# tpoisonooo/how-to-optimize-gemm

Hardware: NVIDIA B200
Metric: SGEMM GFLOP/s (square N=4096 point of the 256..4096 sweep) (higher is better)
Workload: dtype f16x2(scaled split-f32)

## Files before the change

### how-to-optimize-gemm_b200/csrc/capi.cu

```cuda
#include "../../include/b200gemm.h"

#include <cuda.h>
#include <cuda_runtime.h>
#include <stdio.h>
#include <stdlib.h>
#include <string.h>

#include <atomic>
#include <mutex>
#include <vector>

#include "gemm_ffma.cuh"
#include "gemm_generic.cuh"
#include "gemm_mxf4.cuh"
#include "gemm_tc.cuh"

using namespace b200;

namespace {

std::atomic<unsigned long long> g_launches{0};
int g_split_tail = 1;

struct KernelTimer {
  static constexpr int CAP = 1024;
  bool on = false;
  int n = 0;
  cudaEvent_t ev[CAP][2] = {};
  void begin(cudaStream_t st) {
    if (!on || n >= CAP) return;
    if (!ev[n][0]) { cudaEventCreate(&ev[n][0]); cudaEventCreate(&ev[n][1]); }
    cudaEventRecord(ev[n][0], st);
  }
  void end(cudaStream_t st) {
    if (!on || n >= CAP) return;
    cudaEventRecord(ev[n][1], st);
    n++;
  }
} g_ktimer;
std::atomic<int> g_default_f32_mode{-1};
thread_local const char* t_last_kernel = "none";
struct EpiOpts { int axpby = 0; float alpha = 1.f, beta = 0.f; };
thread_local EpiOpts t_epi;
thread_local int t_sm_reserve = 0;
thread_local int t_dynamic_sched = 0;
int g_dbg_b_lbo = 0, g_dbg_b_sbo = 0;

struct Scratch { void* p = nullptr; size_t bytes = 0; };
struct HostPipe {
  bool ready = false;
  cudaStream_t h2d = nullptr, comp = nullptr, d2h = nullptr;
  cudaEvent_t in[8] = {}, done[8] = {};
  cudaError_t init() {
    if (ready) return cudaSuccess;
    cudaError_t e;
    if ((e = cudaStreamCreateWithFlags(&h2d, cudaStreamNonBlocking)) != cudaSuccess) return e;
    if ((e = cudaStreamCreateWithFlags(&comp, cudaStreamNonBlocking)) != cudaSuccess) return e;
    if ((e = cudaStreamCreateWithFlags(&d2h, cudaStreamNonBlocking)) != cudaSuccess) return e;
    for (int i = 0; i < 8; i++) {
      if ((e = cudaEventCreateWithFlags(&in[i], cudaEventDisableTiming)) != cudaSuccess) return e;
      if ((e = cudaEventCreateWithFlags(&done[i], cudaEventDisableTiming)) != cudaSuccess) return e;
    }
    ready = true;
    return cudaSuccess;
  }
};
struct DevCtx {
  int ok = 0;
  int sms = 0;
  int dev = -1;
  int* flags = nullptr;
  unsigned flag_slot = 0;
  int* sched_counters = nullptr;
  unsigned sched_slot = 0;
  std::mutex ws_mu;
  Scratch ws;
  cudaEvent_t ws_event = nullptr;
  cudaStream_t ws_stream = nullptr;
  bool ws_busy = false;
  unsigned cmax_slot = 0;
  float* cmax_buf = nullptr;
  size_t cmax_cap = 0;
  int cmax_dirty[2] = {0, 0};
  cudaStream_t aux = nullptr;
  cudaEvent_t aux_fork = nullptr, aux_join = nullptr;
  std::mutex host_mu;
  Scratch scr[4];
  HostPipe pipe;
  std::vector<const void*> attr_done;
};
constexpr int kMaxDevices = 64;
DevCtx g_ctx[kMaxDevices];
std::mutex g_mu;

typedef CUresult (*EncodeTiledFn)(CUtensorMap*, CUtensorMapDataType, cuuint32_t, void*,
                                  const cuuint64_t*, const cuuint64_t*, const cuuint32_t*,
                                  const cuuint32_t*, CUtensorMapInterleave, CUtensorMapSwizzle,
                                  CUtensorMapL2promotion, CUtensorMapFloatOOBfill);
EncodeTiledFn g_encode = nullptr;

thread_local DevCtx* t_ctx = nullptr;

int ensure_device() {
  int dev = -1;
  if (cudaGetDevice(&dev) != cudaSuccess || dev < 0 || dev >= kMaxDevices) { cudaGetLastError(); t_ctx = nullptr; return B200_ERR_NO_DEVICE; }
  DevCtx* c = &g_ctx[dev];
  t_ctx = c;
  if (c->ok == 1) return 0;
  std::lock_guard<std::mutex> lk(g_mu);
  if (c->ok == 1) return 0;
  cudaDeviceProp prop;
  if (cudaGetDeviceProperties(&prop, dev) != cudaSuccess) { cudaGetLastError(); c->ok = -1; return B200_ERR_NO_DEVICE; }
  if (prop.major != 10) { c->ok = -1; return B200_ERR_NO_DEVICE; }
  if (!g_encode) {
    void* fn = nullptr;
    cudaDriverEntryPointQueryResult qres;
    if (cudaGetDriverEntryPoint("cuTensorMapEncodeTiled", &fn, cudaEnableDefault, &qres) != cudaSuccess ||
        qres != cudaDriverEntryPointSuccess || !fn) {
      cudaGetLastError();
      c->ok = -1;
      return B200_ERR_NO_DEVICE;
    }
    g_encode = reinterpret_cast<EncodeTiledFn>(fn);
  }
  if (!c->flags) {
    if (cudaMalloc(&c->flags, 16 * 1024 * sizeof(int)) != cudaSuccess || cudaMemset(c->flags, 0, 16 * 1024 * sizeof(int)) != cudaSuccess) {
      cudaGetLastError(); c->flags = nullptr; c->ok = -1; return B200_ERR_NO_DEVICE;
    }
  }
  if (!c->sched_counters) {
    if (cudaMalloc(&c->sched_counters, 64 * sizeof(int)) != cudaSuccess || cudaMemset(c->sched_counters, 0, 64 * sizeof(int)) != cudaSuccess) {
      cudaGetLastError(); c->sched_counters = nullptr; c->ok = -1; return B200_ERR_NO_DEVICE;
    }
  }
  if (!c->ws_event && cudaEventCreateWithFlags(&c->ws_event, cudaEventDisableTiming) != cudaSuccess) {
    cudaGetLastError(); c->ok = -1; return B200_ERR_NO_DEVICE;
  }
  c->dev = dev;
  c->sms = prop.multiProcessorCount;
  c->ok = 1;
  return 0;
}

template <typename Kern>
int ensure_smem_attr(Kern kern, int bytes) {
  const void* key = reinterpret_cast<const void*>(kern);
  {
    std::lock_guard<std::mutex> lk(g_mu);
    for (const void* k : t_ctx->attr_done) if (k == key) return 0;
  }
  cudaError_t e = cudaFuncSetAttribute(kern, cudaFuncAttributeMaxDynamicSharedMemorySize, bytes);
  if (e != cudaSuccess) { cudaGetLastError(); return (int)e; }
  std::lock_guard<std::mutex> lk(g_mu);
  t_ctx->attr_done.push_back(key);
  return 0;
}

struct MapKey {
  const void* ptr; int dtype; unsigned long long d0, d1, ld_bytes; unsigned b0, b1; int swz; int dev;
  bool operator==(const MapKey& o) const {
    return ptr == o.ptr && dtype == o.dtype && d0 == o.d0 && d1 == o.d1 && ld_bytes == o.ld_bytes &&
           b0 == o.b0 && b1 == o.b1 && swz == o.swz && dev == o.dev;
  }
};
struct MapEntry { MapKey key; CUtensorMap map; };
std::vector<MapEntry> g_maps;
size_t g_map_next = 0;
constexpr size_t kMapCache = 64;

int get_map(CUtensorMap* out, const void* ptr, CUtensorMapDataType dt, int elem_bytes,
            unsigned long long inner, unsigned long long rows, unsigned long long ld_bytes,
            unsigned box_inner, unsigned box_rows, int swizzle ) {
  MapKey key{ptr, (int)dt, inner, rows, ld_bytes, box_inner, box_rows, swizzle, t_ctx->dev};
  std::lock_guard<std::mutex> lk(g_mu);
  for (auto& e : g_maps)
    if (e.key == key) { *out = e.map; return 0; }
  cuuint64_t dims[2] = {inner, rows};
  cuuint64_t strides[1] = {ld_bytes};
  cuuint32_t box[2] = {box_inner, box_rows};
  cuuint32_t estr[2] = {1, 1};
  CUtensorMap m;
  CUresult r = g_encode(&m, dt, 2, const_cast<void*>(ptr), dims, strides, box, estr,
                        CU_TENSOR_MAP_INTERLEAVE_NONE,
                        swizzle == 1 ? CU_TENSOR_MAP_SWIZZLE_128B
                        : swizzle == 2 ? CU_TENSOR_MAP_SWIZZLE_128B_ATOM_32B
                        : swizzle == 3 ? CU_TENSOR_MAP_SWIZZLE_64B : CU_TENSOR_MAP_SWIZZLE_NONE,
                        CU_TENSOR_MAP_L2_PROMOTION_L2_256B, CU_TENSOR_MAP_FLOAT_OOB_FILL_NONE);
  (void)elem_bytes;
  if (r != CUDA_SUCCESS) return B200_ERR_TENSORMAP;
  if (g_maps.size() < kMapCache) g_maps.push_back({key, m});
  else { g_maps[g_map_next] = {key, m}; g_map_next = (g_map_next + 1) % kMapCache; }
  *out = m;
  return 0;
}

inline bool aligned16(const void* p) { return (reinterpret_cast<uintptr_t>(p) & 15) == 0; }

int check_args(int m, int n, int k, const void* A, int lda, const void* B, int ldb, const void* C, int ldc) {
  if (m < 0 || n < 0 || k < 0) return B200_ERR_BAD_ARG;
  if (m == 0 || n == 0) return 1;
  if (!C || ldc < n) return B200_ERR_BAD_ARG;
  if (k > 0 && (!A || !B || lda < k || ldb < n)) return B200_ERR_BAD_ARG;
  return 0;
}

int last_launch_status() {
  cudaError_t e = cudaPeekAtLastError();
  if (e != cudaSuccess) { cudaGetLastError(); return (int)e; }
  return 0;
}

int g_pdl = 1;
int g_prepass_fork = 1;
int g_dynamic_sched = 0;
template <typename... KArgs, typename... Args>
cudaError_t launch_pdl(void (*kern)(KArgs...), dim3 grid, dim3 block, size_t smem, cudaStream_t st, int cluster, Args&&... args) {
  cudaLaunchConfig_t cfg = {};
  cfg.gridDim = grid; cfg.blockDim = block; cfg.dynamicSmemBytes = smem; cfg.stream = st;
  cudaLaunchAttribute at[2];
  int n = 0;
  if (cluster > 1) {
    at[n].id = cudaLaunchAttributeClusterDimension;
    at[n].val.clusterDim.x = cluster; at[n].val.clusterDim.y = 1; at[n].val.clusterDim.z = 1;
    n++;
  }
  if (g_pdl) {
    at[n].id = cudaLaunchAttributeProgrammaticStreamSerialization;
    at[n].val.programmaticStreamSerializationAllowed = 1;
    n++;
  }
  cfg.attrs = at; cfg.numAttrs = n;
  return cudaLaunchKernelEx(&cfg, kern, std::forward<Args>(args)...);
}

template <typename T>
int launch_zero(int m, int n, T* C, int ldc, cudaStream_t st) {
  dim3 grid((n + 255) / 256, m < 4096 ? m : 4096);
  fill_zero_kernel<T><<<grid, 256, 0, st>>>(m, n, C, ldc);
  g_launches++;
  t_last_kernel = "fill_zero";
  return last_launch_status();
}

template <typename InT, typename OutT>
int launch_generic(int m, int n, int k, const InT* A, int lda, const InT* B, int ldb, OutT* C, int ldc,
                   int accumulate, cudaStream_t st, const char* name) {
  dim3 grid((n + 63) / 64, (m + 63) / 64);
  gemm_generic_kernel<InT, OutT><<<grid, 256, 0, st>>>(m, n, k, A, lda, B, ldb, C, ldc, accumulate);
  g_launches++;
  t_last_kernel = name;
  return last_launch_status();
}

int launch_generic_requant(int m, int n, int k, const int8_t* A, int lda, const int8_t* B, int ldb, int8_t* C,
                           int ldc, const float* scales, const float* bias, cudaStream_t st) {
  dim3 grid((n + 63) / 64, (m + 63) / 64);
  gemm_generic_kernel<int8_t, int8_t><<<grid, 256, 0, st>>>(m, n, k, A, lda, B, ldb, C, ldc, 0, scales, bias);
  g_launches++;
  t_last_kernel = "generic_s8_requant_64x64";
  return last_launch_status();
}

int g_force_bn = 0;
int g_group_rows = 0;
int g_force_cg = 0;
int g_epi8 = 1;
constexpr int kStreamCDefault = 0;
int g_stream_c = -1;
int g_epi_direct = 0;
int g_ffma_fat = -1;
int g_ffma_halves = 1;

template <int KIND, int BN, int STAGES, typename OutT, class Prod = ProdSingle, int A_ROW_BYTES = 128, int CG = 1, int EPIW = 4>
int launch_tc(int m, int n, int k, const void* A, long long lda, int a_rows_total, int a_plane_rows,
              const void* B, long long ldb, int b_rows_total, int b_plane_rows, void* C, int ldc,
              cudaStream_t st, const char* name, int chunk_k = 0, const float* row_max = nullptr,
              const float* col_max = nullptr, int accumulate = 0) {
  using Cfg = TcConfig<KIND, BN, STAGES, Prod, A_ROW_BYTES, CG, EPIW>;
  using T = KindTraits<KIND>;
  constexpr CUtensorMapDataType dt = KIND == KIND_F16 ? CU_TENSOR_MAP_DATA_TYPE_BFLOAT16
                                   : KIND == KIND_FP16 ? CU_TENSOR_MAP_DATA_TYPE_FLOAT16
                                   : KIND == KIND_TF32 ? CU_TENSOR_MAP_DATA_TYPE_FLOAT32
                                                       : CU_TENSOR_MAP_DATA_TYPE_UINT8;
  CUtensorMap tmA, tmB;
  int rc = get_map(&tmA, A, dt, T::ELEM, k, a_rows_total, (unsigned long long)lda * T::ELEM, Cfg::BK, Cfg::BM,
                   A_ROW_BYTES == 128 ? 1 : 3);
  if (rc) return rc;
  rc = get_map(&tmB, B, dt, T::ELEM, n, b_rows_total, (unsigned long long)ldb * T::ELEM, Cfg::B_BOX_COLS, Cfg::BK,
               T::B_LAYOUT == 1 ? 2 : 1);
  if (rc) return rc;
  TcParams p;
  p.C = C; p.ldc = ldc; p.M = m; p.N = n; p.K = k;
  p.tiles_m = (m + Cfg::TILE_M - 1) / Cfg::TILE_M;
  p.tiles_n = (n + BN - 1) / BN;
  p.group_m = (g_group_rows > 0 ? g_group_rows : 2048) / Cfg::TILE_M;
  if (p.group_m < 1) p.group_m = 1;
  constexpr int OB = OutBytes<OutT>::V;
  p.vec_ok = aligned16(C) && ((long long)ldc * OB) % 16 == 0;
  p.a_plane_rows = a_plane_rows; p.b_plane_rows = b_plane_rows;
  p.chunk_kb = chunk_k > 0 ? (chunk_k + Cfg::BK - 1) / Cfg::BK : (k + Cfg::BK - 1) / Cfg::BK;
  if (p.chunk_kb < 1) p.chunk_kb = 1;
  p.dbg_b_lbo = g_dbg_b_lbo; p.dbg_b_sbo = g_dbg_b_sbo;
  p.row_max = row_max; p.col_max = col_max;
  p.accumulate = accumulate;
  p.axpby = t_epi.axpby; p.alpha = t_epi.alpha; p.beta = t_epi.beta;
  p.epi_direct = g_epi_direct;
  p.stream_c = g_stream_c < 0 ? (g_stream_c = (getenv("B200GEMM_STREAM_C") ? atoi(getenv("B200GEMM_STREAM_C")) : kStreamCDefault)) : g_stream_c;
  auto kern = gemm_tc_kernel<KIND, BN, STAGES, OutT, Prod, A_ROW_BYTES, CG, EPIW>;
  if (int arc = ensure_smem_attr(kern, Cfg::SMEM_BYTES)) return arc;
  int tiles = p.tiles_m * p.tiles_n;
  const int units_max = (t_ctx->sms - t_sm_reserve > 2 * CG ? t_ctx->sms - t_sm_reserve : t_ctx->sms) / CG;
  const int num_kb = (k + Cfg::BK - 1) / Cfg::BK;
  const int rem = tiles % units_max;
  int split = 1;
  if (g_split_tail && OB == 4 && rem > 0) {
    split = units_max / rem;
    if (split > 4) split = 4;
    if (split > num_kb / 8) split = num_kb / 8;
    if (split < 1) split = 1;
    if (rem * CG * Cfg::EPI_WARPS > 1024) split = 1;
  }
  p.halfn = 0;
  if (g_split_tail == 1 && tiles >= units_max && rem > 0 && 2 * rem <= units_max &&
      ((BN / 2 / CG) % Cfg::B_BOX_COLS) == 0 && (BN / 2) % 16 == 0 && (BN / 2) % OutPack<OutT>::COLS == 0) {
    p.halfn = 1;
    split = 1;
  }
  p.split = split;
  p.full_tiles = (split > 1 || p.halfn) ? tiles - rem : tiles;
  p.flags = t_ctx->flags + (t_ctx->flag_slot++ % 16) * 1024;
  p.sched_counter = (g_dynamic_sched || t_dynamic_sched) ? t_ctx->sched_counters + (t_ctx->sched_slot++ % 64) : nullptr;
  if (split > 1) {
    cudaError_t e = cudaMemsetAsync(p.flags, 0, 1024 * sizeof(int), st);
    if (e != cudaSuccess) { cudaGetLastError(); return (int)e; }
  }
  const int items = p.full_tiles + (tiles - p.full_tiles) * (p.halfn ? 2 : split);
  const int units = items < units_max ? items : units_max;
  g_ktimer.begin(st);
  {
    cudaError_t e = launch_pdl(kern, dim3(units * CG), dim3(Cfg::THREADS), Cfg::SMEM_BYTES, st, CG, tmA, tmB, p);
    if (e != cudaSuccess) { cudaGetLastError(); return (int)e; }
  }
  g_ktimer.end(st);
  g_launches++;
  t_last_kernel = name;
  return last_launch_status();
}

int pick_bn(int m, int n, bool allow256, bool allow192 = true) {
  if (g_force_bn == 128 || (g_force_bn == 192 && allow192) || (g_force_bn == 256 && allow256)) return g_force_bn;
  const int cands[3] = {256, 192, 128};
  const double eff[3] = {1.00, 0.97, 0.80};
  int best = 128;
  double best_cost = 1e300;
  const int tm = (m + 127) / 128;
  for (int i = 0; i < 3; i++) {
    if (cands[i] == 256 && !allow256) continue;
    if (cands[i] == 192 && !allow192) continue;
    const long long tiles = (long long)tm * ((n + cands[i] - 1) / cands[i]);
    const long long waves = (tiles + t_ctx->sms - 1) / t_ctx->sms;
    const double cost = (double)waves * (cands[i] / eff[i] + 8.0);
    if (cost < best_cost) { best_cost = cost; best = cands[i]; }
  }
  return best;
}

bool use_pair(int m, int n) {
  if (g_force_cg == 1) return false;
  if (g_force_cg == 2) return m > 128 && n > 128;
  if (m <= 128 || n <= 128) return false;
  const long long tiles = (long long)((m + 255) / 256) * ((n + 255) / 256);
  return tiles * 5 >= (long long)(t_ctx->sms / 2) * 4;
}

#define TC_PLAIN(KIND, OUT, NAME)                                                                     \
  if (use_pair(m, n) && g_epi8)                                                                       \
    return launch_tc<KIND, 256, 6, OUT, ProdSingle, 128, 2, 8>(m, n, k, A, lda, m, 0, B, ldb, k, 0, C, ldc, st, NAME "_2cta_256x256_e8"); \
  if (use_pair(m, n))                                                                                 \
    return launch_tc<KIND, 256, 6, OUT, ProdSingle, 128, 2>(m, n, k, A, lda, m, 0, B, ldb, k, 0, C, ldc, st, NAME "_2cta_256x256"); \
  switch (pick_bn(m, n, true)) {                                                                      \
    case 256: return launch_tc<KIND, 256, 4, OUT>(m, n, k, A, lda, m, 0, B, ldb, k, 0, C, ldc, st, NAME "_128x256"); \
    case 192: return launch_tc<KIND, 192, 5, OUT>(m, n, k, A, lda, m, 0, B, ldb, k, 0, C, ldc, st, NAME "_128x192"); \
    default:  return launch_tc<KIND, 128, 6, OUT>(m, n, k, A, lda, m, 0, B, ldb, k, 0, C, ldc, st, NAME "_128x128"); \
  }

int tc_tf32(int m, int n, int k, const float* A, int lda, const float* B, int ldb, float* C, int ldc, cudaStream_t st, int acc = 0) {
  if (use_pair(m, n) && g_epi8)
    return launch_tc<KIND_TF32, 256, 6, float, ProdSingle, 128, 2, 8>(m, n, k, A, lda, m, 0, B, ldb, k, 0, C, ldc, st, "tc_tf32_2cta_256x256_e8", 0, nullptr, nullptr, acc);
  if (use_pair(m, n))
    return launch_tc<KIND_TF32, 256, 6, float, ProdSingle, 128, 2>(m, n, k, A, lda, m, 0, B, ldb, k, 0, C, ldc, st, "tc_tf32_2cta_256x256", 0, nullptr, nullptr, acc);
  switch (pick_bn(m, n, true)) {
    case 256: return launch_tc<KIND_TF32, 256, 4, float>(m, n, k, A, lda, m, 0, B, ldb, k, 0, C, ldc, st, "tc_tf32_128x256", 0, nullptr, nullptr, acc);
    case 192: return launch_tc<KIND_TF32, 192, 5, float>(m, n, k, A, lda, m, 0, B, ldb, k, 0, C, ldc, st, "tc_tf32_128x192", 0, nullptr, nullptr, acc);
    default:  return launch_tc<KIND_TF32, 128, 6, float>(m, n, k, A, lda, m, 0, B, ldb, k, 0, C, ldc, st, "tc_tf32_128x128", 0, nullptr, nullptr, acc);
  }
}
int tc_bf16_f32(int m, int n, int k, const void* A, int lda, const void* B, int ldb, void* C, int ldc, cudaStream_t st) {
  TC_PLAIN(KIND_F16, float, "tc_bf16")
}
int tc_bf16_bf16(int m, int n, int k, const void* A, int lda, const void* B, int ldb, void* C, int ldc, cudaStream_t st) {
  TC_PLAIN(KIND_F16, bf16_out, "tc_bf16_obf16")
}
int tc_s8(int m, int n, int k, const void* A, int lda, const void* B, int ldb, void* C, int ldc, cudaStream_t st) {
  if (use_pair(m, n) && g_epi8)
    return launch_tc<KIND_I8, 256, 6, int32_t, ProdSingle, 128, 2, 8>(m, n, k, A, lda, m, 0, B, ldb, k, 0, C, ldc, st, "tc_s8_2cta_256x256_e8");
  if (use_pair(m, n))
    return launch_tc<KIND_I8, 256, 6, int32_t, ProdSingle, 128, 2>(m, n, k, A, lda, m, 0, B, ldb, k, 0, C, ldc, st, "tc_s8_2cta_256x256");
  if (pick_bn(m, n, true, false) == 256)
    return launch_tc<KIND_I8, 256, 4, int32_t>(m, n, k, A, lda, m, 0, B, ldb, k, 0, C, ldc, st, "tc_s8_128x256");
  return launch_tc<KIND_I8, 128, 6, int32_t>(m, n, k, A, lda, m, 0, B, ldb, k, 0, C, ldc, st, "tc_s8_128x128");
}

int tc_s8_requant(int m, int n, int k, const void* A, int lda, const void* B, int ldb, void* C, int ldc,
                  const float* scales, const float* bias, cudaStream_t st) {
  if (use_pair(m, n) && g_epi8)
    return launch_tc<KIND_I8, 256, 6, s8_out, ProdSingle, 128, 2, 8>(m, n, k, A, lda, m, 0, B, ldb, k, 0, C, ldc, st, "tc_s8_requant_2cta_256x256_e8", 0, scales, bias);
  if (use_pair(m, n))
    return launch_tc<KIND_I8, 256, 6, s8_out, ProdSingle, 128, 2>(m, n, k, A, lda, m, 0, B, ldb, k, 0, C, ldc, st, "tc_s8_requant_2cta_256x256", 0, scales, bias);
  if (pick_bn(m, n, true, false) == 256)
    return launch_tc<KIND_I8, 256, 4, s8_out>(m, n, k, A, lda, m, 0, B, ldb, k, 0, C, ldc, st, "tc_s8_requant_128x256", 0, scales, bias);
  return launch_tc<KIND_I8, 128, 6, s8_out>(m, n, k, A, lda, m, 0, B, ldb, k, 0, C, ldc, st, "tc_s8_requant_128x128", 0, scales, bias);
}

int g_split_chunk_k[3] = {512, 512, 1024};
int split_ws_reserve(size_t need) {
  DevCtx* c = t_ctx;
  if (c->ws.bytes >= need) return B200_OK;
  size_t want = c->ws.bytes ? 2 * c->ws.bytes : ((size_t)256 << 20);
  if (want < need) want = need;
  if (c->ws.p) { cudaDeviceSynchronize(); cudaFree(c->ws.p); }
  c->ws.p = nullptr; c->ws.bytes = 0; c->ws_busy = false;
  cudaError_t e = cudaMalloc(&c->ws.p, want);
  if (e != cudaSuccess && want > need) { cudaGetLastError(); want = need; e = cudaMalloc(&c->ws.p, want); }
  if (e != cudaSuccess) { cudaGetLastError(); c->ws.p = nullptr; return (int)e; }
  c->ws.bytes = want;
  return B200_OK;
}
void ws_acquire(cudaStream_t st) {
  DevCtx* c = t_ctx;
  if (c->ws_busy && c->ws_stream != st) cudaStreamWaitEvent(st, c->ws_event, 0);
}
void ws_release(cudaStream_t st) {
  DevCtx* c = t_ctx;
  cudaEventRecord(c->ws_event, st);
  c->ws_stream = st;
  c->ws_busy = true;
}

inline long long plane_pitch(int cols) { return ((long long)cols + 7) & ~7LL; }
inline int b_plane_rows(int k) { return (k + 31) & ~31; }

template <int NP>
int launch_split(const SplitJob& ja, const SplitJob& jb, int jobs, cudaStream_t st) {
  const long long wide = jobs == 2 && jb.dld > ja.dld ? jb.dld : ja.dld;
  const int tall = jobs == 2 && jb.plane_rows > ja.plane_rows ? jb.plane_rows : ja.plane_rows;
  const int gx = (int)((wide + 2047) / 2048);
  int gy = (t_ctx->sms * 8 + jobs * gx - 1) / (jobs * gx);
  if (gy > (tall + 1) / 2) gy = (tall + 1) / 2;
  if (gy < 1) gy = 1;
  launch_pdl(split_planes_kernel<NP>, dim3(gx, gy, jobs), dim3(256), 0, st, 1, ja, jb);
  g_launches += 1;
  return last_launch_status();
}

template <int NP>
int gemm_f32_split(int m, int n, int k, const float* A, int lda, const float* B, int ldb, float* C, int ldc,
                   cudaStream_t st, int acc = 0, const uint16_t* prepB = nullptr) {
  const long long pka = plane_pitch(k), pnb = plane_pitch(n);
  const int kp = b_plane_rows(k);
  const size_t a_bytes = (size_t)NP * m * pka * 2, b_bytes = (size_t)NP * kp * pnb * 2;
  const size_t a_off = (a_bytes + 1023) & ~(size_t)1023;
  std::lock_guard<std::mutex> wlk(t_ctx->ws_mu);
  if (int rc = split_ws_reserve(prepB ? a_off : a_off + b_bytes)) return rc;
  ws_acquire(st);
  struct Release { cudaStream_t s; ~Release() { ws_release(s); } } rel{st};
  uint16_t* pA = reinterpret_cast<uint16_t*>(t_ctx->ws.p);
  const uint16_t* pB = prepB ? prepB
                             : reinterpret_cast<uint16_t*>(reinterpret_cast<uint8_t*>(t_ctx->ws.p) + a_off);
  const SplitJob ja{A, lda, m, k, pA, pka, m}, jb{B, ldb, k, n, const_cast<uint16_t*>(pB), pnb, kp};
  int rc = launch_split<NP>(ja, jb, prepB ? 1 : 2, st);
  if (rc) return rc;
  if (use_pair(m, n)) {
    if constexpr (NP == 3)
      return launch_tc<KIND_F16, 256, 4, float, ProdX3, 64, 2>(m, n, k, pA, pka, NP * m, m, pB, pnb, NP * kp, kp, C, ldc, st, "tc_bf16x3_2cta_256x256", g_split_chunk_k[0], nullptr, nullptr, acc);
    else
      return launch_tc<KIND_F16, 256, 6, float, ProdX2, 64, 2>(m, n, k, pA, pka, NP * m, m, pB, pnb, NP * kp, kp, C, ldc, st, "tc_bf16x2_2cta_256x256", g_split_chunk_k[1], nullptr, nullptr, acc);
  }
  const int bn = pick_bn(m, n, NP == 2);
  if constexpr (NP == 3) {
    if (bn == 192)
      return launch_tc<KIND_F16, 192, 3, float, ProdX3, 64>(m, n, k, pA, pka, NP * m, m, pB, pnb, NP * kp, kp, C, ldc, st, "tc_bf16x3_128x192", g_split_chunk_k[0], nullptr, nullptr, acc);
    return launch_tc<KIND_F16, 128, 4, float, ProdX3, 64>(m, n, k, pA, pka, NP * m, m, pB, pnb, NP * kp, kp, C, ldc, st, "tc_bf16x3_128x128", g_split_chunk_k[0], nullptr, nullptr, acc);
  } else {
    if (bn == 256)
      return launch_tc<KIND_F16, 256, 4, float, ProdX2, 64>(m, n, k, pA, pka, NP * m, m, pB, pnb, NP * kp, kp, C, ldc, st, "tc_bf16x2_128x256", g_split_chunk_k[1], nullptr, nullptr, acc);
    if (bn == 192)
      return launch_tc<KIND_F16, 192, 4, float, ProdX2, 64>(m, n, k, pA, pka, NP * m, m, pB, pnb, NP * kp, kp, C, ldc, st, "tc_bf16x2_128x192", g_split_chunk_k[1], nullptr, nullptr, acc);
    return launch_tc<KIND_F16, 128, 6, float, ProdX2, 64>(m, n, k, pA, pka, NP * m, m, pB, pnb, NP * kp, kp, C, ldc, st, "tc_bf16x2_128x128", g_split_chunk_k[1], nullptr, nullptr, acc);
  }
}

struct F16Operand {
  const uint16_t* planes;
  long long pitch;
  int plane_rows;
  const float* maxv;
};
inline long long f16_pitch(int cols) { return ((long long)cols + 7) & ~7LL; }
inline int f16_b_rows(int k) { return (k + 31) & ~31; }

int launch_f16_split_rows(const float* A, long long lda, int rows, int cols, float* rmax, uint16_t* planes,
                          long long pitch, int plane_rows, cudaStream_t st) {
  int blocks = (plane_rows + 7) / 8;
  const int cap = t_ctx->sms * 16;
  if (blocks > cap) blocks = cap;
  if (blocks < 1) blocks = 1;
  if (cols <= 1024) launch_pdl(split_f16_rows_kernel<4>, dim3(blocks), dim3(256), 0, st, 1, A, (long long)lda, rows, cols, rmax, planes, pitch, plane_rows);
  else if (cols <= 2048) launch_pdl(split_f16_rows_kernel<8>, dim3(blocks), dim3(256), 0, st, 1, A, (long long)lda, rows, cols, rmax, planes, pitch, plane_rows);
  else if (cols <= 4096) launch_pdl(split_f16_rows_kernel<16>, dim3(blocks), dim3(256), 0, st, 1, A, (long long)lda, rows, cols, rmax, planes, pitch, plane_rows);
  else launch_pdl(split_f16_rows_kernel<0>, dim3(blocks), dim3(256), 0, st, 1, A, (long long)lda, rows, cols, rmax, planes, pitch, plane_rows);
  g_launches++;
  return last_launch_status();
}

int launch_f16_split_cols(const float* B, long long ldb, int rows, int cols, float* cmax, uint16_t* planes,
                          long long pitch, int plane_rows, float* zero_buf, int zero_n, cudaStream_t st) {
  launch_pdl(col_absmax_kernel, dim3((cols + 1023) / 1024, (rows + 15) / 16), dim3(256), 0, st, 1, B, (long long)ldb, rows, cols,
             reinterpret_cast<unsigned int*>(cmax));
  const int gx = (int)((pitch + 2047) / 2048);
  int gy = (t_ctx->sms * 8 + gx - 1) / gx;
  if (gy > (plane_rows + 1) / 2) gy = (plane_rows + 1) / 2;
  if (gy < 1) gy = 1;
  if (zero_buf && zero_n > gx * 2048) {
    cudaMemsetAsync(zero_buf, 0, (size_t)zero_n * 4, st);
    zero_buf = nullptr;
  }
  launch_pdl(split_f16_cols_kernel, dim3(gx, gy), dim3(256), 0, st, 1, B, (long long)ldb, rows, cols, (const float*)cmax, planes, pitch, plane_rows, zero_buf, zero_n);
  g_launches += 2;
  return last_launch_status();
}

int gemm_f16x2_core(int m, int n, int k, const F16Operand& a, const F16Operand& b, float* C, int ldc, int acc,
                    cudaStream_t st) {
  constexpr int NP = 2;
  if (use_pair(m, n))
    return launch_tc<KIND_FP16, 256, 6, float, ProdX2, 64, 2>(m, n, k, a.planes, a.pitch, NP * a.plane_rows, a.plane_rows,
                                                              b.planes, b.pitch, NP * b.plane_rows, b.plane_rows, C, ldc, st,
                                                              "tc_f16x2_2cta_256x256", g_split_chunk_k[2], a.maxv, b.maxv, acc);
  const int bn = pick_bn(m, n, true);
  if (bn == 256)
    return launch_tc<KIND_FP16, 256, 4, float, ProdX2, 64>(m, n, k, a.planes, a.pitch, NP * a.plane_rows, a.plane_rows,
                                                           b.planes, b.pitch, NP * b.plane_rows, b.plane_rows, C, ldc, st,
                                                           "tc_f16x2_128x256", g_split_chunk_k[2], a.maxv, b.maxv, acc);
  if (bn == 192)
    return launch_tc<KIND_FP16, 192, 4, float, ProdX2, 64>(m, n, k, a.planes, a.pitch, NP * a.plane_rows, a.plane_rows,
                                                           b.planes, b.pitch, NP * b.plane_rows, b.plane_rows, C, ldc, st,
                                                           "tc_f16x2_128x192", g_split_chunk_k[2], a.maxv, b.maxv, acc);
  return launch_tc<KIND_FP16, 128, 6, float, ProdX2, 64>(m, n, k, a.planes, a.pitch, NP * a.plane_rows, a.plane_rows,
                                                         b.planes, b.pitch, NP * b.plane_rows, b.plane_rows, C, ldc, st,
                                                         "tc_f16x2_128x128", g_split_chunk_k[2], a.maxv, b.maxv, acc);
}

int cmax_reserve(int n, float** cur, float** other, int* other_dirty) {
  DevCtx* c = t_ctx;
  if (c->cmax_cap < (size_t)n) {
    size_t cap = c->cmax_cap ? 2 * c->cmax_cap : 16384;
    if (cap < (size_t)n) cap = (size_t)n;
    if (c->cmax_buf) { cudaDeviceSynchronize(); cudaFree(c->cmax_buf); }
    c->cmax_buf = nullptr; c->cmax_cap = 0;
    cudaError_t e = cudaMalloc(&c->cmax_buf, 2 * cap * sizeof(float));
    if (e == cudaSuccess) e = cudaMemset(c->cmax_buf, 0, 2 * cap * sizeof(float));
    if (e != cudaSuccess) { cudaGetLastError(); return (int)e; }
    c->cmax_cap = cap;
    c->cmax_dirty[0] = c->cmax_dirty[1] = 0;
  }
  const unsigned slot = c->cmax_slot++ & 1u;
  *cur = c->cmax_buf + slot * c->cmax_cap;
  *other = c->cmax_buf + (slot ^ 1u) * c->cmax_cap;
  *other_dirty = c->cmax_dirty[slot ^ 1u];
  c->cmax_dirty[slot ^ 1u] = 0;
  c->cmax_dirty[slot] = n;
  return 0;
}

int gemm_f32_split_f16(int m, int n, int k, const float* A, int lda, const float* B, int ldb, float* C, int ldc,
                       cudaStream_t st, int acc = 0, const F16Operand* prepA = nullptr, const F16Operand* prepB = nullptr) {
  constexpr int NP = 2;
  const long long pka = f16_pitch(k), pnb = f16_pitch(n);
  const int kp = f16_b_rows(k);
  const size_t a_bytes = prepA ? 0 : (size_t)NP * m * pka * 2, b_bytes = prepB ? 0 : (size_t)NP * kp * pnb * 2;
  const size_t a_off = (a_bytes + 1023) & ~(size_t)1023;
  const size_t r_off = (a_off + b_bytes + 1023) & ~(size_t)1023;
  const size_t total = r_off + (prepA ? 0 : (size_t)m * 4);
  F16Operand oa, ob;
  if (prepA && prepB) return gemm_f16x2_core(m, n, k, *prepA, *prepB, C, ldc, acc, st);
  std::lock_guard<std::mutex> wlk(t_ctx->ws_mu);
  if (int rc = split_ws_reserve(total)) return rc;
  ws_acquire(st);
  struct Release { cudaStream_t s; ~Release() { ws_release(s); } } rel{st};
  uint8_t* base = reinterpret_cast<uint8_t*>(t_ctx->ws.p);
  DevCtx* c = t_ctx;
  const bool fork = !prepA && !prepB && g_prepass_fork && (double)m * k + (double)k * n >= 4.0e6;
  cudaStream_t sb = st;
  if (fork) {
    if (!c->aux) {
      if (cudaStreamCreateWithFlags(&c->aux, cudaStreamNonBlocking) != cudaSuccess ||
          cudaEventCreateWithFlags(&c->aux_fork, cudaEventDisableTiming) != cudaSuccess ||
          cudaEventCreateWithFlags(&c->aux_join, cudaEventDisableTiming) != cudaSuccess) { cudaGetLastError(); return B200_ERR_NO_DEVICE; }
    }
    cudaEventRecord(c->aux_fork, st);
    cudaStreamWaitEvent(c->aux, c->aux_fork, 0);
    sb = c->aux;
  }
  if (prepB) ob = *prepB;
  else {
    uint16_t* pB = reinterpret_cast<uint16_t*>(base + a_off);
    float *cmax, *other;
    int other_dirty;
    if (int rc = cmax_reserve(n, &cmax, &other, &other_dirty)) return rc;
    if (int rc = launch_f16_split_cols(B, ldb, k, n, cmax, pB, pnb, kp, other, other_dirty, sb)) return rc;
    ob = F16Operand{pB, pnb, kp, cmax};
  }
  if (prepA) oa = *prepA;
  else {
    uint16_t* pA = reinterpret_cast<uint16_t*>(base);
    float* rmax = reinterpret_cast<float*>(base + r_off);
    if (int rc = launch_f16_split_rows(A, lda, m, k, rmax, pA, pka, m, st)) return rc;
    oa = F16Operand{pA, pka, m, rmax};
  }
  if (fork) {
    cudaEventRecord(c->aux_join, c->aux);
    cudaStreamWaitEvent(st, c->aux_join, 0);
  }
  return gemm_f16x2_core(m, n, k, oa, ob, C, ldc, acc, st);
}

int launch_ffma(int m, int n, int k, const float* A, int lda, const float* B, int ldb, float* C, int ldc,
                int accumulate, cudaStream_t st) {
  using Cfg = FfmaCfg;
  CUtensorMap tmA, tmB;
  int rc = get_map(&tmA, A, CU_TENSOR_MAP_DATA_TYPE_FLOAT32, 4, k, m, (unsigned long long)lda * 4, Cfg::BK, Cfg::BM, 1);
  if (rc) return rc;
  rc = get_map(&tmB, B, CU_TENSOR_MAP_DATA_TYPE_FLOAT32, 4, n, k, (unsigned long long)ldb * 4, Cfg::BN, Cfg::BK, 0);
  if (rc) return rc;
  FfmaParams p;
  p.C = C; p.ldc = ldc; p.M = m; p.N = n; p.K = k;
  p.vec_ok = aligned16(C) && (ldc % 4) == 0;
  p.accumulate = accumulate;
  p.tiles_m = (m + Cfg::BM - 1) / Cfg::BM;
  p.tiles_n = (n + Cfg::BN - 1) / Cfg::BN;
  p.group_m = 8;
  const int tiles = p.tiles_m * p.tiles_n, slots = 2 * t_ctx->sms;
  const int rem = tiles % slots;
  const bool halves = g_ffma_halves && rem > 0 && 2 * rem <= slots;
  p.full_tiles = halves ? tiles - rem : tiles;
  const int ctas = p.full_tiles + 2 * (tiles - p.full_tiles);
  if (int arc = ensure_smem_attr(gemm_ffma_kernel, Cfg::SMEM_BYTES)) return arc;
  g_ktimer.begin(st);
  gemm_ffma_kernel<<<ctas, Cfg::THREADS, Cfg::SMEM_BYTES, st>>>(tmA, tmB, p);
  g_ktimer.end(st);
  g_launches++;
  t_last_kernel = "ffma_128x128x32_tma";
  return last_launch_status();
}

int launch_ffma_fat(int m, int n, int k, const float* A, int lda, const float* B, int ldb, float* C, int ldc,
                int accumulate, cudaStream_t st) {
  using Cfg = FfmaFatCfg;
  CUtensorMap tmA, tmB;
  int rc = get_map(&tmA, A, CU_TENSOR_MAP_DATA_TYPE_FLOAT32, 4, k, m, (unsigned long long)lda * 4, Cfg::BK, Cfg::BM, 1);
  if (rc) return rc;
  rc = get_map(&tmB, B, CU_TENSOR_MAP_DATA_TYPE_FLOAT32, 4, n, k, (unsigned long long)ldb * 4, Cfg::BN, Cfg::BK, 0);
  if (rc) return rc;
  FfmaParams p;
  p.C = C; p.ldc = ldc; p.M = m; p.N = n; p.K = k;
  p.vec_ok = aligned16(C) && (ldc % 4) == 0;
  p.accumulate = accumulate;
  p.tiles_m = (m + Cfg::BM - 1) / Cfg::BM;
  p.tiles_n = (n + Cfg::BN - 1) / Cfg::BN;
  p.group_m = 8;
  const int tiles = p.tiles_m * p.tiles_n, slots = t_ctx->sms;
  const int rem = tiles % slots;
  const bool halves = g_ffma_halves && rem > 0 && 2 * rem <= slots;
  p.full_tiles = halves ? tiles - rem : tiles;
  const int ctas = p.full_tiles + 2 * (tiles - p.full_tiles);
  if (int arc = ensure_smem_attr(gemm_ffma_fat_kernel, Cfg::SMEM_BYTES)) return arc;
  g_ktimer.begin(st);
  gemm_ffma_fat_kernel<<<ctas, Cfg::THREADS, Cfg::SMEM_BYTES, st>>>(tmA, tmB, p);
  g_ktimer.end(st);
  g_launches++;
  t_last_kernel = "ffma_fat_128x256x32_tma";
  return last_launch_status();
}

bool tma_ok(const void* A, int lda, const void* B, int ldb, int elem) {
  return aligned16(A) && aligned16(B) && ((long long)lda * elem) % 16 == 0 && ((long long)ldb * elem) % 16 == 0;
}

int resolve_f32_mode(int mode) {
  if (mode == B200_F32_AUTO) {
    int d = g_default_f32_mode.load();
    if (d < 0) {
      const char* e = getenv("B200GEMM_F32_MODE");
      d = e ? atoi(e) : B200_F32_F16X2;
      if (d < 0 || d == B200_F32_AUTO || d > B200_F32_F16X2) d = B200_F32_F16X2;
      g_default_f32_mode.store(d);
    }
    return d;
  }
  return mode;
}

int gemm_f32_impl(int m, int n, int k, const float* dA, int lda, const float* dB, int ldb, float* dC,
                  int ldc, int mode, int accumulate, cudaStream_t st) {
  int rc = check_args(m, n, k, dA, lda, dB, ldb, dC, ldc);
  if (rc == 1) return 0;
  if (rc) return rc;
  rc = ensure_device();
  if (rc) return rc;
  if (k == 0) return accumulate ? 0 : launch_zero<float>(m, n, dC, ldc, st);
  const bool was_auto = mode == B200_F32_AUTO;
  mode = resolve_f32_mode(mode);
  const bool tma = tma_ok(dA, lda, dB, ldb, 4);
  if (was_auto && (mode == B200_F32_BF16X3 || mode == B200_F32_F16X2) && tma && (double)m * n * k <= 2.0e8) mode = B200_F32_STRICT;
  else if (was_auto && mode == B200_F32_F16X2 && (double)m * n * k < 1.3e9) mode = B200_F32_BF16X3;
  switch (mode) {
    case B200_F32_STRICT:
      if (tma && (g_ffma_fat == 1 || (g_ffma_fat < 0 && (long long)((m + 127) / 128) * ((n + 255) / 256) >= 96)))
        return launch_ffma_fat(m, n, k, dA, lda, dB, ldb, dC, ldc, accumulate, st);
      if (tma) return launch_ffma(m, n, k, dA, lda, dB, ldb, dC, ldc, accumulate, st);
      return launch_generic<float, float>(m, n, k, dA, lda, dB, ldb, dC, ldc, accumulate, st, "generic_f32_64x64");
    case B200_F32_TF32:
      if (!tma) return launch_generic<float, float>(m, n, k, dA, lda, dB, ldb, dC, ldc, accumulate, st, "generic_f32_64x64");
      return tc_tf32(m, n, k, dA, lda, dB, ldb, dC, ldc, st, accumulate);
    case B200_F32_BF16X3:
      return gemm_f32_split<3>(m, n, k, dA, lda, dB, ldb, dC, ldc, st, accumulate);
    case B200_F32_BF16X2:
      return gemm_f32_split<2>(m, n, k, dA, lda, dB, ldb, dC, ldc, st, accumulate);
    case B200_F32_F16X2:
      return gemm_f32_split_f16(m, n, k, dA, lda, dB, ldb, dC, ldc, st, accumulate);
    default:
      return B200_ERR_UNSUPPORTED;
  }
}

}

extern "C" {

const char* b200_gemm_version(void) { return "b200gemm 0.2 (sm_100a; tcgen05+TMA; round 2)"; }

int b200_gemm_device_ok(void) { return ensure_device(); }

const char* b200_gemm_strerror(int code) {
  switch (code) {
    case B200_OK: return "ok";
    case B200_ERR_BAD_ARG: return "bad argument";
    case B200_ERR_NO_DEVICE: return "no usable sm_100 CUDA device (there is no CPU fallback)";
    case B200_ERR_UNSUPPORTED: return "mode not supported for these operands";
    case B200_ERR_TENSORMAP: return "cuTensorMapEncodeTiled failed";
    case B200_ERR_NCCL: return "NCCL failure (b200_nccl_last_error has the text)";
    default: return code > 0 ? cudaGetErrorString((cudaError_t)code) : "unknown";
  }
}

const char* b200_gemm_last_kernel(void) { return t_last_kernel; }
unsigned long long b200_gemm_launch_count(void) { return g_launches.load(); }
int b200_gemm_default_f32_mode(void) { return resolve_f32_mode(B200_F32_AUTO); }
void b200_gemm_set_default_f32_mode(int mode) {
  if (mode >= 0 && mode != B200_F32_AUTO && mode <= B200_F32_F16X2) g_default_f32_mode.store(mode);
}
void b200_gemm_debug_set_b_desc(int lbo_bytes, int sbo_bytes) { g_dbg_b_lbo = lbo_bytes; g_dbg_b_sbo = sbo_bytes; }
void b200_gemm_debug_set_bn(int bn) { g_force_bn = bn; }
void b200_gemm_debug_set_pdl(int v) { g_pdl = (v & 1) != 0; g_prepass_fork = (v & 2) == 0; }
void b200_gemm_debug_set_dynamic_sched(int on) { g_dynamic_sched = on != 0; }
void b200_gemm_debug_set_cta_group(int cg) { g_force_cg = cg; }
void b200_gemm_debug_set_split_tail(int on) { g_split_tail = on; }
void b200_gemm_debug_set_epilogue(int v) { g_epi_direct = v & 1; g_epi8 = ((v >> 1) & 1) ^ 1; }
void b200_gemm_debug_set_group_rows(int rows) { g_group_rows = rows; }
void b200_gemm_debug_set_ffma_variant(int v) { g_ffma_halves = v & 1; g_ffma_fat = v < 0 ? -1 : (v >> 1) & 1; }
void b200_gemm_debug_set_split_chunk(int x3_k, int x2_k) { g_split_chunk_k[0] = x3_k; g_split_chunk_k[1] = x2_k; g_split_chunk_k[2] = x2_k; }
void b200_gemm_debug_kernel_timing(int enable) { g_ktimer.on = enable != 0; g_ktimer.n = 0; }
int b200_gemm_debug_kernel_time_ms(double* sum_ms) {
  double sum = 0;
  int cnt = 0;
  for (int i = 0; i < g_ktimer.n; i++) {
    float ms = 0.f;
    if (cudaEventSynchronize(g_ktimer.ev[i][1]) == cudaSuccess &&
        cudaEventElapsedTime(&ms, g_ktimer.ev[i][0], g_ktimer.ev[i][1]) == cudaSuccess) { sum += ms; cnt++; }
  }
  cudaGetLastError();
  g_ktimer.n = 0;
  if (sum_ms) *sum_ms = sum;
  return cnt;
}

int b200_gemm_reserve_workspace(size_t bytes) {
  int rc = ensure_device();
  if (rc) return rc;
  std::lock_guard<std::mutex> wlk(t_ctx->ws_mu);
  return split_ws_reserve(bytes);
}
size_t b200_gemm_workspace_bytes(int m, int n, int k, int precision_mode) {
  const int mode = resolve_f32_mode(precision_mode);
  const int np = mode == B200_F32_BF16X3 ? 3 : (mode == B200_F32_BF16X2 || mode == B200_F32_F16X2) ? 2 : 0;
  if (!np || m <= 0 || n <= 0 || k <= 0) return 0;
  const size_t a = ((size_t)np * m * plane_pitch(k) * 2 + 1023) & ~(size_t)1023;
  const size_t b = ((size_t)np * b_plane_rows(k) * plane_pitch(n) * 2 + 1023) & ~(size_t)1023;
  return a + b + (size_t)m * 4 + 1024;
}

int b200_gemm_f32(int m, int n, int k, const float* dA, int lda, const float* dB, int ldb, float* dC,
                  int ldc, int precision_mode, void* stream) {
  return gemm_f32_impl(m, n, k, dA, lda, dB, ldb, dC, ldc, precision_mode, 0, (cudaStream_t)stream);
}

int b200_gemm_f32_ex(int m, int n, int k, float alpha, const float* dA, int lda, const float* dB, int ldb, float beta,
                     float* dC, int ldc, int precision_mode, void* stream) {
  cudaStream_t st = (cudaStream_t)stream;
  if (alpha == 1.f && beta == 0.f) return gemm_f32_impl(m, n, k, dA, lda, dB, ldb, dC, ldc, precision_mode, 0, st);
  if (alpha == 1.f && beta == 1.f) return gemm_f32_impl(m, n, k, dA, lda, dB, ldb, dC, ldc, precision_mode, 1, st);
  int rc = check_args(m, n, k, dA, lda, dB, ldb, dC, ldc);
  if (rc == 1) return 0;
  if (rc) return rc;
  rc = ensure_device();
  if (rc) return rc;
  const int mode = resolve_f32_mode(precision_mode);
  const bool cuda_core = mode == B200_F32_STRICT || !tma_ok(dA, lda, dB, ldb, 4) || k == 0 ||
                         (precision_mode == B200_F32_AUTO && (double)m * n * k <= 2.0e8);
  const dim3 sg((n + 255) / 256, m < 4096 ? m : 4096);
  if (alpha == 0.f || cuda_core) {
    if (alpha == 0.f || k == 0) {
      if (beta == 0.f) return launch_zero<float>(m, n, dC, ldc, st);
      scale_inplace_kernel<<<sg, 256, 0, st>>>(m, n, dC, ldc, beta);
      g_launches++;
      return last_launch_status();
    }
    if (beta != 0.f && beta != alpha) { scale_inplace_kernel<<<sg, 256, 0, st>>>(m, n, dC, ldc, beta / alpha); g_launches++; }
    rc = gemm_f32_impl(m, n, k, dA, lda, dB, ldb, dC, ldc, cuda_core && mode != B200_F32_STRICT && tma_ok(dA, lda, dB, ldb, 4) ? B200_F32_STRICT : mode,
                       beta != 0.f ? 1 : 0, st);
    if (rc) return rc;
    scale_inplace_kernel<<<sg, 256, 0, st>>>(m, n, dC, ldc, alpha);
    g_launches++;
    return last_launch_status();
  }
  t_epi.axpby = 1; t_epi.alpha = alpha; t_epi.beta = beta;
  rc = gemm_f32_impl(m, n, k, dA, lda, dB, ldb, dC, ldc, mode, 0, st);
  t_epi = EpiOpts();
  return rc;
}

int b200_gemm_f32_acc(int m, int n, int k, const float* dA, int lda, const float* dB, int ldb, float* dC,
                      int ldc, int precision_mode, void* stream) {
  return gemm_f32_impl(m, n, k, dA, lda, dB, ldb, dC, ldc, precision_mode, 1, (cudaStream_t)stream);
}

int b200_gemm_bf16(int m, int n, int k, const uint16_t* dA, int lda, const uint16_t* dB, int ldb,
                   void* dC, int ldc, int out_type, void* stream) {
  cudaStream_t st = (cudaStream_t)stream;
  if (out_type != B200_OUT_F32 && out_type != B200_OUT_BF16) return B200_ERR_BAD_ARG;
  int rc = check_args(m, n, k, dA, lda, dB, ldb, dC, ldc);
  if (rc == 1) return 0;
  if (rc) return rc;
  rc = ensure_device();
  if (rc) return rc;
  if (k == 0)
    return out_type == B200_OUT_F32 ? launch_zero<float>(m, n, (float*)dC, ldc, st)
                                    : launch_zero<uint16_t>(m, n, (uint16_t*)dC, ldc, st);
  if (!tma_ok(dA, lda, dB, ldb, 2)) {
    if (out_type == B200_OUT_F32)
      return launch_generic<uint16_t, float>(m, n, k, dA, lda, dB, ldb, (float*)dC, ldc, 0, st, "generic_bf16_64x64");
    return launch_generic<uint16_t, uint16_t>(m, n, k, dA, lda, dB, ldb, (uint16_t*)dC, ldc, 0, st, "generic_bf16_64x64");
  }
  if (out_type == B200_OUT_F32) return tc_bf16_f32(m, n, k, dA, lda, dB, ldb, dC, ldc, st);
  return tc_bf16_bf16(m, n, k, dA, lda, dB, ldb, dC, ldc, st);
}

int b200_gemm_s8s32(int m, int n, int k, const int8_t* dA, int lda, const int8_t* dB, int ldb,
                    int32_t* dC, int ldc, void* stream) {
  cudaStream_t st = (cudaStream_t)stream;
  int rc = check_args(m, n, k, dA, lda, dB, ldb, dC, ldc);
  if (rc == 1) return 0;
  if (rc) return rc;
  rc = ensure_device();
  if (rc) return rc;
  if (k == 0) return launch_zero<int32_t>(m, n, dC, ldc, st);
  if (!tma_ok(dA, lda, dB, ldb, 1))
    return launch_generic<int8_t, int32_t>(m, n, k, dA, lda, dB, ldb, dC, ldc, 0, st, "generic_s8_64x64");
  return tc_s8(m, n, k, dA, lda, dB, ldb, dC, ldc, st);
}

struct b200_packed {
  int side;
  int rows, cols, mode, np, plane_rows;
  long long pitch;
  uint16_t* planes;
  float* maxv;
  int dev;
};
struct b200_packed_a : b200_packed {};
struct b200_packed_b : b200_packed {};

static int pack_operand(int side, int rows, int cols, const float* d, int ld, int precision_mode, b200_packed* h,
                        cudaStream_t st) {
  if (rows <= 0 || cols <= 0 || !d || ld < cols) return B200_ERR_BAD_ARG;
  const int mode = resolve_f32_mode(precision_mode);
  if (mode != B200_F32_F16X2 && (side != 1 || (mode != B200_F32_BF16X3 && mode != B200_F32_BF16X2))) return B200_ERR_UNSUPPORTED;
  int rc = ensure_device();
  if (rc) return rc;
  h->side = side; h->rows = rows; h->cols = cols; h->mode = mode; h->planes = nullptr; h->maxv = nullptr;
  h->dev = t_ctx->dev;
  if (mode == B200_F32_F16X2) {
    h->np = 2;
    h->pitch = f16_pitch(cols);
    h->plane_rows = side == 0 ? rows : f16_b_rows(rows);
    const size_t nmax = side == 0 ? (size_t)rows : (size_t)cols;
    cudaError_t e = cudaMalloc(&h->planes, (size_t)2 * h->plane_rows * h->pitch * 2);
    if (e == cudaSuccess) e = cudaMalloc(&h->maxv, nmax * 4);
    if (e != cudaSuccess) { cudaGetLastError(); return (int)e; }
    if (side == 0) return launch_f16_split_rows(d, ld, rows, cols, h->maxv, h->planes, h->pitch, h->plane_rows, st);
    e = cudaMemsetAsync(h->maxv, 0, nmax * 4, st);
    if (e != cudaSuccess) { cudaGetLastError(); return (int)e; }
    return launch_f16_split_cols(d, ld, rows, cols, h->maxv, h->planes, h->pitch, h->plane_rows, nullptr, 0, st);
  }
  h->np = mode == B200_F32_BF16X3 ? 3 : 2;
  h->pitch = plane_pitch(cols);
  h->plane_rows = b_plane_rows(rows);
  cudaError_t e = cudaMalloc(&h->planes, (size_t)h->np * h->plane_rows * h->pitch * 2);
  if (e != cudaSuccess) { cudaGetLastError(); return (int)e; }
  const SplitJob jb{d, ld, rows, cols, h->planes, h->pitch, h->plane_rows};
  return h->np == 3 ? launch_split<3>(jb, jb, 1, st) : launch_split<2>(jb, jb, 1, st);
}
static void pack_release(b200_packed* h) {
  if (!h) return;
  if (h->planes) cudaFree(h->planes);
  if (h->maxv) cudaFree(h->maxv);
}

int b200_gemm_f32_pack_b(int k, int n, const float* dB, int ldb, int precision_mode, b200_packed_b** out,
                         void* stream) {
  if (!out) return B200_ERR_BAD_ARG;
  *out = nullptr;
  b200_packed_b* h = new b200_packed_b();
  int rc = pack_operand(1, k, n, dB, ldb, precision_mode, h, (cudaStream_t)stream);
  t_last_kernel = "split_planes";
  if (rc) { pack_release(h); delete h; return rc; }
  *out = h;
  return B200_OK;
}

int b200_gemm_f32_pack_a(int m, int k, const float* dA, int lda, int precision_mode, b200_packed_a** out,
                         void* stream) {
  if (!out) return B200_ERR_BAD_ARG;
  *out = nullptr;
  b200_packed_a* h = new b200_packed_a();
  int rc = pack_operand(0, m, k, dA, lda, precision_mode, h, (cudaStream_t)stream);
  t_last_kernel = "split_planes";
  if (rc) { pack_release(h); delete h; return rc; }
  *out = h;
  return B200_OK;
}

static int gemm_packed_impl(int m, int n, int k, const float* dA, int lda, const b200_packed* pa, int a_k0,
                            const b200_packed* pb, float* dC, int ldc, int accumulate, cudaStream_t st) {
  if (!pb || pb->rows != k || pb->cols != n) return B200_ERR_BAD_ARG;
  if (pa && (pa->rows != m || a_k0 < 0 || a_k0 + k > pa->cols || (a_k0 & 7) || pa->mode != pb->mode)) return B200_ERR_BAD_ARG;
  int rc = check_args(m, n, k, pa ? (const void*)pa->planes : (const void*)dA, pa ? k : lda, pb->planes, n, dC, ldc);
  if (rc == 1) return 0;
  if (rc) return rc;
  rc = ensure_device();
  if (rc) return rc;
  if (pb->dev != t_ctx->dev || (pa && pa->dev != t_ctx->dev)) return B200_ERR_BAD_ARG;
  if (pb->mode == B200_F32_F16X2) {
    const F16Operand ob{pb->planes, pb->pitch, pb->plane_rows, pb->maxv};
    if (pa) {
      const F16Operand oa{pa->planes + a_k0, pa->pitch, pa->plane_rows, pa->maxv};
      return gemm_f32_split_f16(m, n, k, nullptr, 0, nullptr, 0, dC, ldc, st, accumulate ? 1 : 0, &oa, &ob);
    }
    return gemm_f32_split_f16(m, n, k, dA, lda, nullptr, 0, dC, ldc, st, accumulate ? 1 : 0, nullptr, &ob);
  }
  if (pa) return B200_ERR_UNSUPPORTED;
  return pb->np == 3 ? gemm_f32_split<3>(m, n, k, dA, lda, nullptr, 0, dC, ldc, st, accumulate ? 1 : 0, pb->planes)
                     : gemm_f32_split<2>(m, n, k, dA, lda, nullptr, 0, dC, ldc, st, accumulate ? 1 : 0, pb->planes);
}

int b200_gemm_f32_packed(int m, int n, int k, const float* dA, int lda, const b200_packed_b* pb, float* dC,
                         int ldc, int accumulate, void* stream) {
  return gemm_packed_impl(m, n, k, dA, lda, nullptr, 0, pb, dC, ldc, accumulate, (cudaStream_t)stream);
}

int b200_gemm_f32_packed_ab(int m, int n, int k, const b200_packed_a* pa, int a_k0, const b200_packed_b* pb,
                            float* dC, int ldc, int accumulate, void* stream) {
  if (!pa) return B200_ERR_BAD_ARG;
  return gemm_packed_impl(m, n, k, nullptr, 0, pa, a_k0, pb, dC, ldc, accumulate, (cudaStream_t)stream);
}

void b200_gemm_f32_pack_free(b200_packed_b* pb) {
  if (!pb) return;
  pack_release(pb);
  delete pb;
}
void b200_gemm_f32_pack_free_a(b200_packed_a* pa) {
  if (!pa) return;
  pack_release(pa);
  delete pa;
}

int b200_gemm_s8s8_requant(int m, int n, int k, const int8_t* dA, int lda, const int8_t* dB, int ldb,
                           int8_t* dC, int ldc, const float* dScales, const float* dBias, void* stream) {
  cudaStream_t st = (cudaStream_t)stream;
  int rc = check_args(m, n, k, dA, lda, dB, ldb, dC, ldc);
  if (rc == 1) return 0;
  if (rc) return rc;
  if (!dScales) return B200_ERR_BAD_ARG;
  rc = ensure_device();
  if (rc) return rc;
  if (k == 0 || !tma_ok(dA, lda, dB, ldb, 1))
    return launch_generic_requant(m, n, k, dA, lda, dB, ldb, dC, ldc, dScales, dBias, st);
  return tc_s8_requant(m, n, k, dA, lda, dB, ldb, dC, ldc, dScales, dBias, st);
}

size_t b200_mxf4_q_bytes(int rows, int k) { return rows <= 0 || k <= 0 ? 0 : (size_t)rows * (size_t)(((k + 127) & ~127) / 2); }
size_t b200_mxf4_sf_bytes(int rows, int k) {
  return rows <= 0 || k <= 0 ? 0 : (size_t)((rows + 127) / 128) * (size_t)((k + 127) / 128) * 512;
}

int b200_mxf4_quantize_a(int m, int k, const float* dA, int lda, uint8_t* dQ, uint8_t* dSF, void* stream) {
  if (m <= 0 || k <= 0 || !dA || !dQ || !dSF || lda < k) return B200_ERR_BAD_ARG;
  int rc = ensure_device();
  if (rc) return rc;
  const int kpad = (k + 127) & ~127, rows_pad = (m + 127) & ~127;
  const long long total = (long long)rows_pad * (kpad / 32);
  long long blocks = (total + 255) / 256;
  if (blocks > t_ctx->sms * 16) blocks = t_ctx->sms * 16;
  mxf4_quantize_rows_kernel<<<(unsigned)blocks, 256, 0, (cudaStream_t)stream>>>(dA, lda, m, k, dQ, kpad, dSF, rows_pad);
  g_launches++;
  t_last_kernel = "mxf4_quantize_rows";
  return last_launch_status();
}

int b200_mxf4_quantize_b(int k, int n, const float* dB, int ldb, uint8_t* dQ, uint8_t* dSF, void* stream) {
  if (n <= 0 || k <= 0 || !dB || !dQ || !dSF || ldb < n) return B200_ERR_BAD_ARG;
  int rc = ensure_device();
  if (rc) return rc;
  const int kpad = (k + 127) & ~127, n_pad = (n + 127) & ~127;
  mxf4_quantize_cols_t_kernel<<<dim3((n_pad + 255) / 256, kpad / 32), 256, 0, (cudaStream_t)stream>>>(dB, ldb, k, n, dQ, kpad, dSF, n_pad);
  g_launches++;
  t_last_kernel = "mxf4_quantize_cols_t";
  return last_launch_status();
}

int b200_gemm_mxf4(int m, int n, int k, const uint8_t* dAq, const uint8_t* dSFA, const uint8_t* dBq, const uint8_t* dSFB,
                   float* dC, int ldc, void* stream) {
  if (m < 0 || n < 0 || k < 0) return B200_ERR_BAD_ARG;
  if (m == 0 || n == 0) return 0;
  if (!dC || ldc < n) return B200_ERR_BAD_ARG;
  int rc = ensure_device();
  if (rc) return rc;
  cudaStream_t st = (cudaStream_t)stream;
  if (k == 0) return launch_zero<float>(m, n, dC, ldc, st);
  if (!dAq || !dSFA || !dBq || !dSFB || !aligned16(dAq) || !aligned16(dBq) || !aligned16(dSFA) || !aligned16(dSFB)) return B200_ERR_BAD_ARG;
  using Cfg = Mxf4Cfg<128>;
  const int kpad = (k + 127) & ~127;
  CUtensorMap tmA, tmB;
  rc = get_map(&tmA, dAq, CU_TENSOR_MAP_DATA_TYPE_UINT8, 1, kpad / 2, m, kpad / 2, 128, Cfg::BM, 1);
  if (rc) return rc;
  rc = get_map(&tmB, dBq, CU_TENSOR_MAP_DATA_TYPE_UINT8, 1, kpad / 2, n, kpad / 2, 128, 128, 1);
  if (rc) return rc;
  Mxf4Params p;
  p.C = dC; p.ldc = ldc; p.M = m; p.N = n; p.K = kpad;
  p.sfa = dSFA; p.sfb = dSFB;
  p.tiles_m = (m + 127) / 128; p.tiles_n = (n + 127) / 128;
  p.vec_ok = aligned16(dC) && (ldc % 4) == 0;
  auto kern = gemm_mxf4_kernel<128>;
  if (int arc = ensure_smem_attr(kern, Cfg::SMEM_BYTES)) return arc;
  const int tiles = p.tiles_m * p.tiles_n;
  g_ktimer.begin(st);
  kern<<<tiles < t_ctx->sms ? tiles : t_ctx->sms, Cfg::THREADS, Cfg::SMEM_BYTES, st>>>(tmA, tmB, p);
  g_ktimer.end(st);
  g_launches++;
  t_last_kernel = "tc_mxf4_128x128";
  return last_launch_status();
}

int b200_convert_f32_to_bf16(const float* dSrc, uint16_t* dDst, size_t count, void* stream) {
  if (count == 0) return 0;
  if (!dSrc || !dDst) return B200_ERR_BAD_ARG;
  int rc = ensure_device();
  if (rc) return rc;
  size_t blocks = (count + 255) / 256;
  if (blocks > 148 * 32) blocks = 148 * 32;
  convert_f32_to_bf16_kernel<<<(unsigned)blocks, 256, 0, (cudaStream_t)stream>>>(dSrc, dDst, count);
  g_launches++;
  t_last_kernel = "convert_f32_to_bf16";
  return last_launch_status();
}

namespace {
cudaError_t scratch(int i, size_t bytes, void** out) {
  Scratch* scr = t_ctx->scr;
  if (scr[i].bytes < bytes) {
    if (scr[i].p) cudaFree(scr[i].p);
    scr[i].p = nullptr; scr[i].bytes = 0;
    cudaError_t e = cudaMalloc(&scr[i].p, bytes);
    if (e != cudaSuccess) return e;
    scr[i].bytes = bytes;
  }
  *out = scr[i].p;
  return cudaSuccess;
}
}

#define CK(x) do { cudaError_t e_ = (x); if (e_ != cudaSuccess) { cudaGetLastError(); return (int)e_; } } while (0)

int b200_gemm_f32_host(int m, int n, int k, const float* A, int lda, const float* B, int ldb, float* C,
                       int ldc, int precision_mode) {
  int rc = check_args(m, n, k, A, lda, B, ldb, C, ldc);
  if (rc == 1) return 0;
  if (rc) return rc;
  rc = ensure_device();
  if (rc) return rc;
  std::lock_guard<std::mutex> lk(t_ctx->host_mu);
  float *dA = nullptr, *dB = nullptr, *dC = nullptr;
  const int mode = precision_mode;
  const int pk = (k + 3) & ~3, pn = (n + 3) & ~3;
  const size_t pa = (size_t)pk * 4, pb = (size_t)pn * 4, pc = (size_t)pn * 4;
  if (k > 0) {
    CK(scratch(0, pa * m, (void**)&dA));
    CK(scratch(1, pb * k, (void**)&dB));
  }
  CK(scratch(2, pc * m, (void**)&dC));
  const int blocks = (k > 0 && m >= 2048 && (double)m * n * k >= 8.0e9) ? 4 : 1;
  if (blocks == 1) {
    cudaStream_t st = 0;
    if (k > 0) {
      CK(cudaMemcpy2DAsync(dA, pa, A, (size_t)lda * 4, (size_t)k * 4, m, cudaMemcpyHostToDevice, st));
      CK(cudaMemcpy2DAsync(dB, pb, B, (size_t)ldb * 4, (size_t)n * 4, k, cudaMemcpyHostToDevice, st));
    }
    CK(cudaMemcpy2DAsync(dC, pc, C, (size_t)ldc * 4, (size_t)n * 4, m, cudaMemcpyHostToDevice, st));
    rc = gemm_f32_impl(m, n, k, dA, pk, dB, pn, dC, pn, mode, 1, st);
    if (rc) return rc;
    CK(cudaMemcpy2DAsync(C, (size_t)ldc * 4, dC, pc, (size_t)n * 4, m, cudaMemcpyDeviceToHost, st));
    CK(cudaStreamSynchronize(st));
    return 0;
  }
  CK(t_ctx->pipe.init());
  CK(cudaMemcpy2DAsync(dB, pb, B, (size_t)ldb * 4, (size_t)n * 4, k, cudaMemcpyHostToDevice, t_ctx->pipe.h2d));
  const int rows_per = ((m + blocks - 1) / blocks + 255) & ~255;
  int nb = 0;
  for (int r0 = 0; r0 < m; r0 += rows_per, nb++) {
    const int rows = m - r0 < rows_per ? m - r0 : rows_per;
    float* dAi = dA + (size_t)r0 * pk;
    float* dCi = dC + (size_t)r0 * pn;
    CK(cudaMemcpy2DAsync(dAi, pa, A + (size_t)r0 * lda, (size_t)lda * 4, (size_t)k * 4, rows, cudaMemcpyHostToDevice, t_ctx->pipe.h2d));
    CK(cudaMemcpy2DAsync(dCi, pc, C + (size_t)r0 * ldc, (size_t)ldc * 4, (size_t)n * 4, rows, cudaMemcpyHostToDevice, t_ctx->pipe.h2d));
    CK(cudaEventRecord(t_ctx->pipe.in[nb], t_ctx->pipe.h2d));
    CK(cudaStreamWaitEvent(t_ctx->pipe.comp, t_ctx->pipe.in[nb], 0));
    rc = gemm_f32_impl(rows, n, k, dAi, pk, dB, pn, dCi, pn, mode, 1, t_ctx->pipe.comp);
    if (rc) return rc;
    CK(cudaEventRecord(t_ctx->pipe.done[nb], t_ctx->pipe.comp));
    CK(cudaStreamWaitEvent(t_ctx->pipe.d2h, t_ctx->pipe.done[nb], 0));
    CK(cudaMemcpy2DAsync(C + (size_t)r0 * ldc, (size_t)ldc * 4, dCi, pc, (size_t)n * 4, rows, cudaMemcpyDeviceToHost, t_ctx->pipe.d2h));
  }
  CK(cudaStreamSynchronize(t_ctx->pipe.d2h));
  CK(cudaStreamSynchronize(t_ctx->pipe.comp));
  return 0;
}

int b200_gemm_s8s32_host(int m, int n, int k, const int8_t* A, int lda, const int8_t* B, int ldb,
                         int32_t* C, int ldc) {
  int rc = check_args(m, n, k, A, lda, B, ldb, C, ldc);
  if (rc == 1) return 0;
  if (rc) return rc;
  rc = ensure_device();
  if (rc) return rc;
  std::lock_guard<std::mutex> lk(t_ctx->host_mu);
  int8_t *dA = nullptr, *dB = nullptr;
  int32_t* dC = nullptr;
  const size_t pa = ((size_t)k + 15) & ~(size_t)15, pb = ((size_t)n + 15) & ~(size_t)15;
  const size_t pc = (size_t)n * 4;
  cudaStream_t st = 0;
  if (k > 0) {
    CK(scratch(0, pa * m, (void**)&dA));
    CK(scratch(1, pb * k, (void**)&dB));
    CK(cudaMemcpy2DAsync(dA, pa, A, (size_t)lda, (size_t)k, m, cudaMemcpyHostToDevice, st));
    CK(cudaMemcpy2DAsync(dB, pb, B, (size_t)ldb, (size_t)n, k, cudaMemcpyHostToDevice, st));
  }
  CK(scratch(2, pc * m, (void**)&dC));
  rc = b200_gemm_s8s32(m, n, k, dA, (int)pa, dB, (int)pb, dC, n, st);
  if (rc) return rc;
  CK(cudaMemcpy2DAsync(C, (size_t)ldc * 4, dC, pc, pc, m, cudaMemcpyDeviceToHost, st));
  CK(cudaStreamSynchronize(st));
  return 0;
}

}

#include "rowpanel.cuh"
```

### how-to-optimize-gemm_b200/csrc/gemm_tc.cuh

```cuda
#pragma once
#include <cuda_fp16.h>
#include <string.h>
#include <type_traits>

#include "ptx.cuh"

namespace b200 {

template <int KIND> struct KindTraits;
template <> struct KindTraits<KIND_F16>  { static constexpr int ELEM = 2, UMMA_K = 16, AB_FMT = 1, C_FMT = 1, B_LAYOUT = 2, B_SBO = 1024; };
template <> struct KindTraits<KIND_TF32> { static constexpr int ELEM = 4, UMMA_K = 8,  AB_FMT = 2, C_FMT = 1, B_LAYOUT = 1, B_SBO = 512; };
template <> struct KindTraits<KIND_FP16> { static constexpr int ELEM = 2, UMMA_K = 16, AB_FMT = 0, C_FMT = 1, B_LAYOUT = 2, B_SBO = 1024; };
template <> struct KindTraits<KIND_I8>   { static constexpr int ELEM = 1, UMMA_K = 32, AB_FMT = 1, C_FMT = 2, B_LAYOUT = 2, B_SBO = 1024; };

struct ProdSingle {
  static constexpr int N = 1, NPA = 1, NPB = 1;
  __host__ __device__ static constexpr int ia(int) { return 0; }
  __host__ __device__ static constexpr int ib(int) { return 0; }
};
struct ProdX3 {
  static constexpr int N = 6, NPA = 3, NPB = 3;
  __host__ __device__ static constexpr int ia(int i) { return i == 1 ? 2 : (i == 2 || i == 4) ? 1 : 0; }
  __host__ __device__ static constexpr int ib(int i) { return i == 0 ? 2 : (i == 2 || i == 3) ? 1 : 0; }
};
struct ProdX2 {
  static constexpr int N = 3, NPA = 2, NPB = 2;
  __host__ __device__ static constexpr int ia(int i) { return i == 1 ? 1 : 0; }
  __host__ __device__ static constexpr int ib(int i) { return i == 0 ? 1 : 0; }
};

struct TcParams {
  void* C;
  long long ldc;
  int M, N, K;
  int tiles_m, tiles_n;
  int group_m;
  int vec_ok;
  int a_plane_rows;
  int b_plane_rows;
  int chunk_kb;
  int full_tiles, split;
  int halfn;
  int* flags;
  int* sched_counter;
  const float* row_max;
  const float* col_max;
  float alpha, beta;
  int axpby;
  int accumulate;
  int stream_c;
  int epi_direct;
  int dbg_b_lbo, dbg_b_sbo;
};

template <int KIND, int BN, int STAGES, class Prod, int A_ROW_BYTES, int CG = 1, int EPIW = 4>
struct TcConfig {
  using T = KindTraits<KIND>;
  static constexpr bool REGACC = Prod::N > 1;
  static constexpr int EPI_WARPS = REGACC ? 8 : EPIW;
  static constexpr int EPI_WARP0 = REGACC ? 4 : 2;
  static constexpr int BM = 128;
  static constexpr int BK = A_ROW_BYTES / T::ELEM;
  static constexpr int A_PLANE = BM * A_ROW_BYTES;
  static constexpr int A_LAYOUT = A_ROW_BYTES == 128 ? 2 : 4;
  static constexpr int A_SBO = 8 * A_ROW_BYTES;
  static constexpr int B_BOX_COLS = 128 / T::ELEM;
  static constexpr int BN_CTA = BN / CG;
  static constexpr int B_BOXES = BN_CTA / B_BOX_COLS;
  static constexpr int B_BOX_BYTES = BK * 128;
  static constexpr int B_PLANE = B_BOXES * B_BOX_BYTES;
  static constexpr int A_STAGE = Prod::NPA * A_PLANE;
  static constexpr int B_STAGE = Prod::NPB * B_PLANE;
  static constexpr int STAGE_BYTES = A_STAGE + B_STAGE;
  static constexpr int TX_BYTES = CG * STAGE_BYTES;
  static constexpr int MMAS_PER_STAGE = BK / T::UMMA_K;
  static constexpr int A_KADV = T::UMMA_K * T::ELEM;
  static constexpr int B_KADV = T::UMMA_K * 128;
  static constexpr int EPI_STAGING = EPI_WARPS * 32 * 128;
  static constexpr int ACC_STRIDE = BN <= 128 ? 128 : 256;
  static constexpr int TMEM_COLS = 2 * ACC_STRIDE;
  static constexpr int SCHED_SLOTS = 8;
  static constexpr int SCHED_WARP = REGACC ? 2 : EPI_WARP0 + EPI_WARPS;
  static constexpr int NUM_BARS = 2 * STAGES + 4 + 2 * SCHED_SLOTS + 1;
  static constexpr int SMEM_BYTES = 1024  + STAGES * STAGE_BYTES + EPI_STAGING +
                                    NUM_BARS * 8 + 16 + 4 * SCHED_SLOTS;
  static constexpr int THREADS = 32 * (EPI_WARP0 + EPI_WARPS + (REGACC ? 0 : 1));
  static_assert(!REGACC || BN % 64 == 0, "register accumulation splits the tile columns over two warp sets of 32-column groups");
  static_assert(SMEM_BYTES <= 232448, "exceeds the 227 KB dynamic shared memory of sm_100");
  static_assert(BN_CTA % B_BOX_COLS == 0 && BN % 16 == 0 && BN <= 256, "invalid BN");
  static constexpr int TILE_M = 128 * CG;
};

__device__ __forceinline__ void tile_coords(int t, int tiles_m, int tiles_n, int group_m, int& mb,
                                            int& nb) {
  const int per_group = group_m * tiles_n;
  const int g = t / per_group;
  const int first_m = g * group_m;
  const int rows = min(group_m, tiles_m - first_m);
  const int r = t - g * per_group;
  mb = first_m + r % rows;
  nb = r / rows;
}

__host__ __device__ __forceinline__ int pow2_exp(float maxv) {
  uint32_t bits;
#ifdef __CUDA_ARCH__
  bits = __float_as_uint(maxv);
#else
  memcpy(&bits, &maxv, 4);
#endif
  const int ef = (int)((bits >> 23) & 0xFF);
  return (ef == 0 || ef == 255) ? 0 : ef - 126;
}
__device__ __forceinline__ float exp2i(int e) { return __uint_as_float((uint32_t)(127 + e) << 23); }
__device__ __forceinline__ float mul_pow2(float x, int e) {
  const int h = e >> 1;
  return x * exp2i(h) * exp2i(min(e - h, 127));
}

struct WorkItem { int tile, part, kb0, kb1, nsub, bn; };
template <int BN>
__device__ __forceinline__ WorkItem work_item(int w, const TcParams& p, int num_kb) {
  WorkItem it;
  it.nsub = 0; it.bn = BN;
  if (w < p.full_tiles) { it.tile = w; it.part = 0; it.kb0 = 0; it.kb1 = num_kb; return it; }
  const int r = w - p.full_tiles;
  if (p.halfn) {
    it.tile = p.full_tiles + (r >> 1); it.nsub = r & 1; it.bn = BN / 2;
    it.part = 0; it.kb0 = 0; it.kb1 = num_kb;
    return it;
  }
  it.tile = p.full_tiles + r / p.split;
  it.part = r - (r / p.split) * p.split;
  it.kb0 = (int)((long long)num_kb * it.part / p.split);
  it.kb1 = (int)((long long)num_kb * (it.part + 1) / p.split);
  return it;
}

struct TileSched {
  int slot;
  uint32_t phase;
  int w;
  __device__ __forceinline__ int next(int lane, bool dynamic, bool pair, uint32_t bar_sfull, uint32_t sempty_leader,
                                      const volatile int* items, int step, int num_items, uint32_t gate = 0) {
    if (!dynamic) {
      const int r = w;
      w += step;
      return r < num_items ? r : -1;
    }
    mbar_wait_cluster(bar_sfull + 8 * slot, phase);
    const int r = items[slot];
    __syncwarp();
    if (lane == 0) {
      if (pair) mbar_arrive_cluster(sempty_leader + 8 * slot);
      else mbar_arrive(sempty_leader + 8 * slot);
      if (gate) mbar_arrive(gate);
    }
    if (++slot == 8) { slot = 0; phase ^= 1; }
    return r;
  }
};

template <typename OutT> struct OutPack;
template <> struct OutPack<float> {
  static constexpr int COLS = 32;
  __device__ static void pack(const uint32_t (&a)[32], const uint32_t (&)[32], uint32_t (&w)[32]) {
#pragma unroll
    for (int i = 0; i < 32; i++) w[i] = a[i];
  }
};
template <> struct OutPack<int32_t> {
  static constexpr int COLS = 32;
  __device__ static void pack(const uint32_t (&a)[32], const uint32_t (&)[32], uint32_t (&w)[32]) {
#pragma unroll
    for (int i = 0; i < 32; i++) w[i] = a[i];
  }
};
struct bf16_out {};
template <> struct OutPack<bf16_out> {
  static constexpr int COLS = 64;
  __device__ static uint32_t cvt2(uint32_t lo, uint32_t hi) {
    uint32_t r;
    asm("cvt.rn.bf16x2.f32 %0, %1, %2;" : "=r"(r) : "f"(__uint_as_float(hi)), "f"(__uint_as_float(lo)));
    return r;
  }
  __device__ static void pack(const uint32_t (&a)[32], const uint32_t (&b)[32], uint32_t (&w)[32]) {
#pragma unroll
    for (int i = 0; i < 16; i++) w[i] = cvt2(a[2 * i], a[2 * i + 1]);
#pragma unroll
    for (int i = 0; i < 16; i++) w[16 + i] = cvt2(b[2 * i], b[2 * i + 1]);
  }
};
struct s8_out {};
template <> struct OutPack<s8_out> {
  static constexpr int COLS = 32;
  __device__ static void pack(const uint32_t (&)[32], const uint32_t (&)[32], uint32_t (&)[32]) {}
};
template <typename OutT> struct OutBytes { static constexpr int V = 4; };
template <> struct OutBytes<bf16_out> { static constexpr int V = 2; };
template <> struct OutBytes<s8_out> { static constexpr int V = 1; };

template <int CG, int SLOTS>
__device__ __forceinline__ void run_tile_scheduler(const TcParams& p, int lane, int num_items, int num_units,
                                                   uint32_t bar_sfull, uint32_t bar_sempty, uint32_t s_items, uint32_t bar_gate) {
  int slot = 0;
  uint32_t ph = 0, gph = 0;
  const int total = num_items + num_units;
  for (int i = 0;; i++) {
    if (i > 0) {
      mbar_wait(bar_gate, gph);
      gph ^= 1;
    }
    mbar_wait_cluster(bar_sempty + 8 * slot, ph ^ 1);
    int w = 0;
    if (lane == 0) {
      w = atomicAdd(p.sched_counter, 1);
      if (w == total - 1) atomicExch(p.sched_counter, 0);
      const uint32_t item = (uint32_t)(w < num_items ? w : -1);
#pragma unroll
      for (int r = 0; r < CG; r++) {
        st_shared_cluster_u32(mapa(s_items + 4 * slot, r), item);
        mbar_arrive_cluster(mapa(bar_sfull + 8 * slot, r));
      }
    }
    w = __shfl_sync(0xffffffffu, w, 0);
    if (w >= num_items) break;
    if (++slot == SLOTS) { slot = 0; ph ^= 1; }
  }
}

template <int KIND, int BN, int STAGES, typename OutT, class Prod, int A_ROW_BYTES, int CG, int EPIW>
__global__ void __launch_bounds__((TcConfig<KIND, BN, STAGES, Prod, A_ROW_BYTES, CG, EPIW>::THREADS), 1)
gemm_tc_kernel(const __grid_constant__ CUtensorMap tmA, const __grid_constant__ CUtensorMap tmB,
               const TcParams p) {
  using Cfg = TcConfig<KIND, BN, STAGES, Prod, A_ROW_BYTES, CG, EPIW>;
  using T = KindTraits<KIND>;
  constexpr int OB = OutBytes<OutT>::V;

  extern __shared__ uint8_t smem_raw[];
  const uint32_t smem_base = (smem_u32(smem_raw) + 1023u) & ~1023u;
  const uint32_t sA = smem_base;
  const uint32_t sB = sA + STAGES * Cfg::A_STAGE;
  const uint32_t sEpi = sB + STAGES * Cfg::B_STAGE;
  const uint32_t sBar = sEpi + Cfg::EPI_STAGING;
  const uint32_t bar_full = sBar;
  const uint32_t bar_empty = sBar + 8 * STAGES;
  const uint32_t bar_tfull = sBar + 16 * STAGES;
  const uint32_t bar_tempty = bar_tfull + 16;
  const uint32_t s_tmem_ptr = bar_tempty + 16;
  const uint32_t bar_sfull = s_tmem_ptr + 16;
  const uint32_t bar_sempty = bar_sfull + 8 * Cfg::SCHED_SLOTS;
  const uint32_t bar_gate = bar_sempty + 8 * Cfg::SCHED_SLOTS;
  const uint32_t s_items = bar_gate + 8;
  uint8_t* smem_gen = smem_raw + (smem_base - smem_u32(smem_raw));

  const int warp = threadIdx.x >> 5;
  const int lane = threadIdx.x & 31;
  const uint32_t cta_rank = CG == 2 ? cluster_ctarank() : 0u;
  const bool leader = cta_rank == 0;
  const int unit = CG == 2 ? (int)(blockIdx.x >> 1) : (int)blockIdx.x;
  const int num_units = CG == 2 ? (int)(gridDim.x >> 1) : (int)gridDim.x;

  if (warp == 0 && lane == 0) {
    tma_prefetch_desc(&tmA);
    tma_prefetch_desc(&tmB);
    for (int i = 0; i < STAGES; i++) {
      mbar_init(bar_full + 8 * i, 1);
      mbar_init(bar_empty + 8 * i, 1);
    }
    for (int i = 0; i < 2; i++) {
      mbar_init(bar_tfull + 8 * i, 1);
      mbar_init(bar_tempty + 8 * i, Cfg::EPI_WARPS * CG);
    }
    for (int i = 0; i < Cfg::SCHED_SLOTS; i++) {
      mbar_init(bar_sfull + 8 * i, 1);
      mbar_init(bar_sempty + 8 * i, CG * (1 + Cfg::EPI_WARPS) + 1);
    }
    mbar_init(bar_gate, 1);
    fence_barrier_init();
  }
  if (warp == 1) {
    if constexpr (CG == 2) tmem_alloc_cg2<Cfg::TMEM_COLS>(s_tmem_ptr);
    else tmem_alloc<Cfg::TMEM_COLS>(s_tmem_ptr);
  }
  tc_fence_before();
  if constexpr (CG == 2) cluster_sync(); else __syncthreads();
  tc_fence_after();
  const uint32_t tmem_base = *reinterpret_cast<volatile uint32_t*>(smem_gen + (s_tmem_ptr - smem_base));
  griddep_launch();
  griddep_wait();

  const int num_tiles = p.tiles_m * p.tiles_n;
  const int num_items = p.full_tiles + (num_tiles - p.full_tiles) * (p.halfn ? 2 : p.split);
  const int num_kb = (p.K + Cfg::BK - 1) / Cfg::BK;
  TileSched sched;
  sched.slot = 0; sched.phase = 0; sched.w = unit;
  const bool dyn = p.sched_counter != nullptr;
#define NEXT_ITEM_G(GATE) sched.next(lane, dyn, CG == 2, bar_sfull, CG == 2 ? mapa(bar_sempty, 0) : bar_sempty, \
                                     reinterpret_cast<const volatile int*>(smem_gen + (s_items - smem_base)), num_units, num_items, GATE)
#define NEXT_ITEM() NEXT_ITEM_G(0u)

  if (warp < Cfg::EPI_WARP0) {
  if constexpr (Cfg::REGACC) setmaxnreg_dec<88>();
  if (warp == 0) {
    {
      int s = 0;
      uint32_t ph = 0;
      const uint32_t gate = leader ? bar_gate : 0u;
      for (int w = NEXT_ITEM_G(gate); w >= 0; w = NEXT_ITEM_G(gate)) {
        const WorkItem it = work_item<BN>(w, p, num_kb);
        int mb, nb;
        tile_coords(it.tile, p.tiles_m, p.tiles_n, p.group_m, mb, nb);
        const int bn_cta = it.bn / CG;
        const int boxes = bn_cta / Cfg::B_BOX_COLS;
        const uint32_t tx_bytes = CG * (Cfg::A_STAGE + Prod::NPB * boxes * Cfg::B_BOX_BYTES);
        const int m0 = mb * Cfg::TILE_M + (int)cta_rank * Cfg::BM, n0 = nb * BN + it.nsub * it.bn + (int)cta_rank * bn_cta;
        for (int kb = it.kb0; kb < it.kb1; kb++) {
          mbar_wait(bar_empty + 8 * s, ph ^ 1);
          const uint32_t full = CG == 2 ? mapa(bar_full + 8 * s, 0) : bar_full + 8 * s;
          if (elect_one()) {
          if (leader) mbar_arrive_expect_tx(bar_full + 8 * s, tx_bytes);
#pragma unroll
          for (int pa = 0; pa < Prod::NPA; pa++) {
            const uint32_t dst = sA + s * Cfg::A_STAGE + pa * Cfg::A_PLANE;
            if constexpr (CG == 2) tma_load_2d_cg2(dst, &tmA, full, kb * Cfg::BK, pa * p.a_plane_rows + m0);
            else tma_load_2d(dst, &tmA, full, kb * Cfg::BK, pa * p.a_plane_rows + m0);
          }
#pragma unroll
          for (int pb = 0; pb < Prod::NPB; pb++)
#pragma unroll
            for (int j = 0; j < Cfg::B_BOXES; j++) {
              if (j >= boxes) break;
              const uint32_t dst = sB + s * Cfg::B_STAGE + pb * Cfg::B_PLANE + j * Cfg::B_BOX_BYTES;
              if constexpr (CG == 2)
                tma_load_2d_cg2(dst, &tmB, full, n0 + j * Cfg::B_BOX_COLS, pb * p.b_plane_rows + kb * Cfg::BK);
              else
                tma_load_2d(dst, &tmB, full, n0 + j * Cfg::B_BOX_COLS, pb * p.b_plane_rows + kb * Cfg::BK);
            }
          }
          __syncwarp();
          if (++s == STAGES) { s = 0; ph ^= 1; }
        }
      }
    }
  } else if (warp == 1) {
    if (leader) {
      const uint32_t b_lbo = p.dbg_b_lbo ? (uint32_t)p.dbg_b_lbo : (uint32_t)Cfg::B_BOX_BYTES;
      const uint32_t b_sbo = p.dbg_b_sbo ? (uint32_t)p.dbg_b_sbo : (uint32_t)T::B_SBO;
      int s = 0;
      uint32_t ph = 0;
      int as = 0;
      uint32_t aph = 0;
      for (int w = NEXT_ITEM(); w >= 0; w = NEXT_ITEM()) {
       const WorkItem it = work_item<BN>(w, p, num_kb);
       const uint32_t idesc = make_idesc(T::C_FMT, T::AB_FMT, 0, 1, Cfg::TILE_M, it.bn);
       for (int c0 = it.kb0; c0 < it.kb1; c0 += p.chunk_kb) {
        mbar_wait(bar_tempty + 8 * as, aph ^ 1);
        tc_fence_after();
        const uint32_t d_tmem = tmem_base + as * Cfg::ACC_STRIDE;
        const int c1 = min(c0 + p.chunk_kb, it.kb1);
        for (int kb = c0; kb < c1; kb++) {
          mbar_wait(bar_full + 8 * s, ph);
          tc_fence_after();
          const uint32_t a0 = sA + s * Cfg::A_STAGE;
          const uint32_t b0 = sB + s * Cfg::B_STAGE;
          if (elect_one()) {
#pragma unroll
          for (int pr = 0; pr < Prod::N; pr++) {
#pragma unroll
            for (int k = 0; k < Cfg::MMAS_PER_STAGE; k++) {
              const uint64_t ad = make_sdesc(a0 + Prod::ia(pr) * Cfg::A_PLANE + k * Cfg::A_KADV, 16,
                                             Cfg::A_SBO, Cfg::A_LAYOUT);
              const uint64_t bd = make_sdesc(b0 + Prod::ib(pr) * Cfg::B_PLANE + k * Cfg::B_KADV, b_lbo,
                                             b_sbo, T::B_LAYOUT);
              if constexpr (CG == 2) tc_mma_cg2<KIND>(d_tmem, ad, bd, idesc, ((kb - c0) | k | pr) != 0 ? 1u : 0u);
              else tc_mma<KIND>(d_tmem, ad, bd, idesc, ((kb - c0) | k | pr) != 0 ? 1u : 0u);
            }
          }
          if constexpr (CG == 2) tc_commit_cg2(bar_empty + 8 * s, 3); else tc_commit(bar_empty + 8 * s);
          }
          __syncwarp();
          if (++s == STAGES) { s = 0; ph ^= 1; }
        }
        if (elect_one()) {
          if constexpr (CG == 2) tc_commit_cg2(bar_tfull + 8 * as, 3); else tc_commit(bar_tfull + 8 * as);
        }
        __syncwarp();
        if (++as == 2) { as = 0; aph ^= 1; }
       }
      }
    }
  } else if (Cfg::REGACC && warp == Cfg::SCHED_WARP) {
    if (dyn && leader)
      run_tile_scheduler<CG, Cfg::SCHED_SLOTS>(p, lane, num_items, num_units, bar_sfull, bar_sempty, s_items, bar_gate);
  }
  } else if (!Cfg::REGACC && warp == Cfg::SCHED_WARP) {
    if (dyn && leader)
      run_tile_scheduler<CG, Cfg::SCHED_SLOTS>(p, lane, num_items, num_units, bar_sfull, bar_sempty, s_items, bar_gate);
  } else {
   if constexpr (Cfg::REGACC) {
    setmaxnreg_inc<208>();
    const int ew = warp - Cfg::EPI_WARP0;
    const int q = ew & 3;
    const int half = ew >> 2;
    uint8_t* stg = smem_gen + (sEpi - smem_base) + ew * 4096;
    constexpr int HC = BN / 2;
    constexpr int NJ = HC / 32;
    int as = 0;
    uint32_t aph = 0;
    const uint32_t tempty_base = CG == 2 ? mapa(bar_tempty, 0) : bar_tempty;
    for (int w = NEXT_ITEM(); w >= 0; w = NEXT_ITEM()) {
      const WorkItem it = work_item<BN>(w, p, num_kb);
      int mb, nb;
      tile_coords(it.tile, p.tiles_m, p.tiles_n, p.group_m, mb, nb);
      const int hc = it.bn / 2;
      const int nj = hc / 32;
      const int m0 = mb * Cfg::TILE_M + (int)cta_rank * Cfg::BM + q * 32;
      const int n0 = nb * BN + it.nsub * it.bn + half * hc;
      const uint32_t t_col = (uint32_t)(half * hc);
      float acc[NJ][32];
      const int my_re = (p.row_max != nullptr && m0 + lane < p.M) ? pow2_exp(__ldg(p.row_max + m0 + lane)) : 0;
      bool first = true;
      for (int c0 = it.kb0; c0 < it.kb1; c0 += p.chunk_kb) {
        mbar_wait(bar_tfull + 8 * as, aph);
        tc_fence_after();
        const uint32_t t_addr = tmem_base + ((uint32_t)(q * 32) << 16) + as * Cfg::ACC_STRIDE + t_col;
#pragma unroll
        for (int j = 0; j < NJ; j++) {
          if (j < nj) {
            uint32_t r[32];
            tmem_ld_32x32b_x32(t_addr + j * 32, r);
            tmem_ld_wait();
            if (first) {
#pragma unroll
              for (int i = 0; i < 32; i++) acc[j][i] = __uint_as_float(r[i]);
            } else {
#pragma unroll
              for (int i = 0; i < 32; i++) acc[j][i] = __fadd_rn(acc[j][i], __uint_as_float(r[i]));
            }
          }
        }
        first = false;
        tc_fence_before();
        __syncwarp();
        if (lane == 0) {
          if constexpr (CG == 2) mbar_arrive_cluster(tempty_base + 8 * as);
          else mbar_arrive(bar_tempty + 8 * as);
        }
        if (++as == 2) { as = 0; aph ^= 1; }
      }
      int* flag = p.flags + ((it.tile - p.full_tiles) * CG + (int)cta_rank) * Cfg::EPI_WARPS + ew;
      if (it.part > 0) {
        if (lane == 0) {
          const long long t0 = clock64();
          while (true) {
            int v;
            asm volatile("ld.acquire.gpu.global.s32 %0, [%1];" : "=r"(v) : "l"(flag) : "memory");
            if (v == it.part) break;
            if (clock64() - t0 > 4000000000LL) { asm volatile("trap;"); }
          }
        }
        __syncwarp();
      }
      const bool fold = p.accumulate != 0 || it.part > 0 || (p.axpby && p.beta != 0.f);
      const float al = p.axpby ? p.alpha : 1.f;
      const float be = (p.axpby && it.part == 0) ? p.beta : 1.f;
      const int chunk = lane & 7;
#pragma unroll
      for (int j = 0; j < NJ; j++) {
        if (j < nj) {
          const int col = n0 + j * 32 + chunk * 4;
          const bool vec = p.vec_ok && col + 4 <= p.N;
          int ce[4] = {0, 0, 0, 0};
          if (p.col_max != nullptr) {
#pragma unroll
            for (int e = 0; e < 4; e++)
              if (col + e < p.N) ce[e] = pow2_exp(__ldg(p.col_max + col + e));
          }
          if (fold && vec) {
#pragma unroll
            for (int i = 0; i < 8; i++) {
              const int gm = m0 + i * 4 + (lane >> 3);
              if (gm < p.M) asm volatile("prefetch.global.L1 [%0];" ::"l"(reinterpret_cast<const float*>(p.C) + (long long)gm * p.ldc + col));
            }
          }
#pragma unroll
          for (int g = 0; g < 8; g++) {
            uint4 v = make_uint4(__float_as_uint(acc[j][4 * g]), __float_as_uint(acc[j][4 * g + 1]),
                                 __float_as_uint(acc[j][4 * g + 2]), __float_as_uint(acc[j][4 * g + 3]));
            *reinterpret_cast<uint4*>(stg + lane * 128 + ((g ^ (lane & 7)) << 4)) = v;
          }
          __syncwarp();
#pragma unroll 1
          for (int i = 0; i < 8; i++) {
            const int row = i * 4 + (lane >> 3);
            const int gm = m0 + row;
            const int re = __shfl_sync(0xffffffffu, my_re, row);
            float4 v = *reinterpret_cast<const float4*>(stg + row * 128 + ((chunk ^ (row & 7)) << 4));
            if (gm < p.M) {
              if (p.row_max != nullptr) {
                v.x = mul_pow2(v.x, re + ce[0]); v.y = mul_pow2(v.y, re + ce[1]);
                v.z = mul_pow2(v.z, re + ce[2]); v.w = mul_pow2(v.w, re + ce[3]);
              }
              float* dst = reinterpret_cast<float*>(p.C) + (long long)gm * p.ldc + col;
              if (p.axpby) { v.x *= al; v.y *= al; v.z *= al; v.w *= al; }
              if (vec) {
                if (fold) {
                  const float4 o = it.part > 0 ? __ldcg(reinterpret_cast<const float4*>(dst)) : *reinterpret_cast<const float4*>(dst);
                  if (p.axpby) { v.x = fmaf(be, o.x, v.x); v.y = fmaf(be, o.y, v.y); v.z = fmaf(be, o.z, v.z); v.w = fmaf(be, o.w, v.w); }
                  else { v.x += o.x; v.y += o.y; v.z += o.z; v.w += o.w; }
                }
                if (p.stream_c) __stcs(reinterpret_cast<float4*>(dst), v);
                else *reinterpret_cast<float4*>(dst) = v;
              } else {
                const float vv[4] = {v.x, v.y, v.z, v.w};
#pragma unroll
                for (int e = 0; e < 4; e++)
                  if (col + e < p.N) dst[e] = !fold ? vv[e] : p.axpby ? fmaf(be, __ldcg(dst + e), vv[e]) : vv[e] + __ldcg(dst + e);
              }
            }
          }
          __syncwarp();
        }
      }
      if (w >= p.full_tiles && p.split > 1) {
        __threadfence();
        __syncwarp();
        if (lane == 0) {
          const int nv = it.part + 1 == p.split ? 0 : it.part + 1;
          asm volatile("st.release.gpu.global.s32 [%0], %1;" ::"l"(flag), "r"(nv) : "memory");
        }
      }
    }
   } else {
    const int q = warp & 3;
    const int ew = warp - Cfg::EPI_WARP0;
    const int ehalf = ew >> 2;
    uint8_t* stg = smem_gen + (sEpi - smem_base) + ew * 4096;
    constexpr int COLS = OutPack<OutT>::COLS;
    constexpr int VEC_ELEMS = 16 / OB;
    int as = 0;
    uint32_t aph = 0;
    const uint32_t tempty_base = CG == 2 ? mapa(bar_tempty, 0) : bar_tempty;
    for (int w = NEXT_ITEM(); w >= 0; w = NEXT_ITEM()) {
      const WorkItem it = work_item<BN>(w, p, num_kb);
      int mb, nb;
      tile_coords(it.tile, p.tiles_m, p.tiles_n, p.group_m, mb, nb);
      const int m0 = mb * Cfg::TILE_M + (int)cta_rank * Cfg::BM + q * 32, n0 = nb * BN + it.nsub * it.bn;
      const int passes = it.bn / COLS;
      float sc = 0.0f, bi = 0.0f;
      bool hb = false;
      if constexpr (std::is_same<OutT, s8_out>::value) {
        hb = p.col_max != nullptr;
        if (m0 + lane < p.M) {
          sc = __ldg(p.row_max + m0 + lane);
          if (hb) bi = __ldg(p.col_max + m0 + lane);
        }
      }
      int* flag = p.flags + ((it.tile - p.full_tiles) * CG + (int)cta_rank) * Cfg::EPI_WARPS + ew;
      if (it.part > 0) {
        if (lane == 0) {
          const long long t0 = clock64();
          while (true) {
            int v;
            asm volatile("ld.acquire.gpu.global.s32 %0, [%1];" : "=r"(v) : "l"(flag) : "memory");
            if (v == it.part) break;
            if (clock64() - t0 > 4000000000LL) { asm volatile("trap;"); }
          }
        }
        __syncwarp();
      }
     for (int c0 = it.kb0; c0 < it.kb1; c0 += p.chunk_kb) {
      const bool fold = p.accumulate != 0 || c0 != it.kb0 || it.part > 0 || (p.axpby && p.beta != 0.f);
      const float al = p.axpby ? p.alpha : 1.f;
      const float be = (p.axpby && it.part == 0 && c0 == it.kb0) ? p.beta : 1.f;
      mbar_wait(bar_tfull + 8 * as, aph);
      tc_fence_after();
      const uint32_t t_addr = tmem_base + ((uint32_t)(q * 32) << 16) + as * Cfg::ACC_STRIDE;
#pragma unroll 1
      const int ps0 = Cfg::EPI_WARPS == 8 ? ehalf * (passes >> 1) : 0;
      const int ps1 = Cfg::EPI_WARPS == 8 ? (ehalf == 0 ? (passes >> 1) : passes) : passes;
      if (ps0 == ps1) {
        tc_fence_before();
        __syncwarp();
        if (lane == 0) {
          if constexpr (CG == 2) mbar_arrive_cluster(tempty_base + 8 * as);
          else mbar_arrive(bar_tempty + 8 * as);
        }
      }
      for (int ps = ps0; ps < ps1; ps++) {
       if constexpr (std::is_same<OutT, s8_out>::value) {
        uint32_t ra[32];
        tmem_ld_32x32b_x32(t_addr + ps * 32, ra);
        tmem_ld_wait();
        if (ps == ps1 - 1) {
          tc_fence_before();
          __syncwarp();
          if (lane == 0) {
            if constexpr (CG == 2) mbar_arrive_cluster(tempty_base + 8 * as);
            else mbar_arrive(bar_tempty + 8 * as);
          }
        }
        const int gm = m0 + lane, col0 = n0 + ps * 32;
        if (gm < p.M && col0 < p.N) {
          uint32_t w8[8];
#pragma unroll
          for (int j = 0; j < 8; j++) {
            uint32_t v = 0;
#pragma unroll
            for (int e = 0; e < 4; e++)
              v |= ((uint32_t)requant_s8((int32_t)ra[4 * j + e], sc, bi, hb) & 0xFFu) << (8 * e);
            w8[j] = v;
          }
          uint8_t* dst = reinterpret_cast<uint8_t*>(p.C) + (long long)gm * p.ldc + col0;
          if (p.vec_ok && col0 + 32 <= p.N) {
            reinterpret_cast<uint4*>(dst)[0] = make_uint4(w8[0], w8[1], w8[2], w8[3]);
            reinterpret_cast<uint4*>(dst)[1] = make_uint4(w8[4], w8[5], w8[6], w8[7]);
          } else {
#pragma unroll
            for (int e = 0; e < 32; e++)
              if (col0 + e < p.N) dst[e] = (uint8_t)(w8[e >> 2] >> (8 * (e & 3)));
          }
        }
       } else {
        const int chunk = lane & 7;
        const int col = n0 + ps * COLS + chunk * VEC_ELEMS;
        const bool vec = p.vec_ok && col + VEC_ELEMS <= p.N;
        float4 old[8];
        if constexpr (OB == 4) {
          if (fold && vec) {
#pragma unroll
            for (int i = 0; i < 8; i++) {
              const int gm = m0 + i * 4 + (lane >> 3);
              old[i] = gm < p.M ? __ldcg(reinterpret_cast<const float4*>(
                                      reinterpret_cast<const float*>(p.C) + (long long)gm * p.ldc + col))
                                : make_float4(0.f, 0.f, 0.f, 0.f);
            }
          }
        }
        uint32_t ra[32], rb[32], w[32];
        tmem_ld_32x32b_x32(t_addr + ps * (COLS == 64 ? 64 : 32), ra);
        if constexpr (COLS == 64) tmem_ld_32x32b_x32(t_addr + ps * 64 + 32, rb);
        tmem_ld_wait();
        if (ps == ps1 - 1) {
          tc_fence_before();
          __syncwarp();
          if (lane == 0) {
            if constexpr (CG == 2) mbar_arrive_cluster(tempty_base + 8 * as);
            else mbar_arrive(bar_tempty + 8 * as);
          }
        }
        OutPack<OutT>::pack(ra, rb, w);
        if (p.epi_direct && !fold && !p.axpby && p.row_max == nullptr && p.vec_ok && n0 + (ps + 1) * COLS <= p.N) {
          const int gm = m0 + lane;
          if (gm < p.M) {
            uint4* dst = reinterpret_cast<uint4*>(reinterpret_cast<uint8_t*>(p.C) +
                                                  ((long long)gm * p.ldc + n0 + ps * COLS) * OB);
#pragma unroll
            for (int j = 0; j < 8; j++) dst[j] = make_uint4(w[4 * j], w[4 * j + 1], w[4 * j + 2], w[4 * j + 3]);
          }
          continue;
        }
#pragma unroll
        for (int j = 0; j < 8; j++) {
          uint4 v = make_uint4(w[4 * j], w[4 * j + 1], w[4 * j + 2], w[4 * j + 3]);
          *reinterpret_cast<uint4*>(stg + lane * 128 + ((j ^ (lane & 7)) << 4)) = v;
        }
        __syncwarp();
#pragma unroll
        for (int i = 0; i < 8; i++) {
          const int row = i * 4 + (lane >> 3);
          const int gm = m0 + row;
          uint4 v = *reinterpret_cast<const uint4*>(stg + row * 128 + ((chunk ^ (row & 7)) << 4));
          if (gm < p.M) {
            uint8_t* dst = reinterpret_cast<uint8_t*>(p.C) + ((long long)gm * p.ldc + col) * OB;
            if (vec) {
              if constexpr (std::is_same<OutT, float>::value) {
                if (p.axpby) {
                  const float4 o = fold ? old[i] : make_float4(0.f, 0.f, 0.f, 0.f);
                  v.x = __float_as_uint(fmaf(be, o.x, al * __uint_as_float(v.x)));
                  v.y = __float_as_uint(fmaf(be, o.y, al * __uint_as_float(v.y)));
                  v.z = __float_as_uint(fmaf(be, o.z, al * __uint_as_float(v.z)));
                  v.w = __float_as_uint(fmaf(be, o.w, al * __uint_as_float(v.w)));
                } else if (fold) {
                  v.x = __float_as_uint(__uint_as_float(v.x) + old[i].x);
                  v.y = __float_as_uint(__uint_as_float(v.y) + old[i].y);
                  v.z = __float_as_uint(__uint_as_float(v.z) + old[i].z);
                  v.w = __float_as_uint(__uint_as_float(v.w) + old[i].w);
                }
              } else if constexpr (std::is_same<OutT, int32_t>::value) {
                if (fold) {
                  v.x += __float_as_uint(old[i].x); v.y += __float_as_uint(old[i].y);
                  v.z += __float_as_uint(old[i].z); v.w += __float_as_uint(old[i].w);
                }
              }
              *reinterpret_cast<uint4*>(dst) = v;
            } else {
              uint32_t vv[4] = {v.x, v.y, v.z, v.w};
              if constexpr (OB == 4) {
#pragma unroll
                for (int e = 0; e < 4; e++)
                  if (col + e < p.N) {
                    if constexpr (std::is_same<OutT, float>::value) {
                      if (p.axpby) vv[e] = __float_as_uint(fmaf(be, fold ? __ldcg(reinterpret_cast<const float*>(dst) + e) : 0.f, al * __uint_as_float(vv[e])));
                      else if (fold) vv[e] = __float_as_uint(__uint_as_float(vv[e]) + __ldcg(reinterpret_cast<const float*>(dst) + e));
                    } else if constexpr (std::is_same<OutT, int32_t>::value) {
                      if (fold) vv[e] += __ldcg(reinterpret_cast<const uint32_t*>(dst) + e);
                    }
                    reinterpret_cast<uint32_t*>(dst)[e] = vv[e];
                  }
              } else {
#pragma unroll
                for (int e = 0; e < 8; e++)
                  if (col + e < p.N)
                    reinterpret_cast<uint16_t*>(dst)[e] = (uint16_t)(vv[e >> 1] >> ((e & 1) * 16));
              }
            }
          }
        }
        __syncwarp();
       }
      }
      if (++as == 2) { as = 0; aph ^= 1; }
     }
      if (w >= p.full_tiles && p.split > 1) {
        __threadfence();
        __syncwarp();
        if (lane == 0) {
          const int nv = it.part + 1 == p.split ? 0 : it.part + 1;
          asm volatile("st.release.gpu.global.s32 [%0], %1;" ::"l"(flag), "r"(nv) : "memory");
        }
      }
    }
  }

  }

#undef NEXT_ITEM
#undef NEXT_ITEM_G
  tc_fence_before();
  if constexpr (CG == 2) cluster_sync(); else __syncthreads();
  if (warp == 1) {
    tc_fence_after();
    if constexpr (CG == 2) tmem_dealloc_cg2<Cfg::TMEM_COLS>(tmem_base);
    else tmem_dealloc<Cfg::TMEM_COLS>(tmem_base);
  }
}

struct SplitJob {
  const float* src; long long ld; int rows, cols;
  uint16_t* dst; long long dld; int plane_rows;
};

template <int NP>
__global__ void __launch_bounds__(256) split_planes_kernel(const SplitJob ja, const SplitJob jb) {
  griddep_launch();
  griddep_wait();
  const SplitJob& jo = blockIdx.z == 0 ? ja : jb;
  const float* __restrict__ src = jo.src;
  uint16_t* __restrict__ dst = jo.dst;
  const long long ld = jo.ld, dld = jo.dld;
  const int rows = jo.rows, cols = jo.cols, plane_rows = jo.plane_rows;
  const int c = (int)(blockIdx.x * 256 + threadIdx.x) * 8;
  if (c >= dld) return;
  const bool vec = c + 8 <= cols && (ld & 3) == 0 && (reinterpret_cast<uintptr_t>(src) & 15) == 0;
  for (int r0 = blockIdx.y * 2; r0 < plane_rows; r0 += gridDim.y * 2) {
    float x[2][8];
#pragma unroll
    for (int u = 0; u < 2; u++) {
      const int r = r0 + u;
#pragma unroll
      for (int e = 0; e < 8; e++) x[u][e] = 0.f;
      if (r < rows) {
        const float* s = src + (long long)r * ld + c;
        if (vec) {
          const float4 v0 = __ldcs(reinterpret_cast<const float4*>(s));
          const float4 v1 = __ldcs(reinterpret_cast<const float4*>(s) + 1);
          x[u][0] = v0.x; x[u][1] = v0.y; x[u][2] = v0.z; x[u][3] = v0.w;
          x[u][4] = v1.x; x[u][5] = v1.y; x[u][6] = v1.z; x[u][7] = v1.w;
        } else {
#pragma unroll
          for (int e = 0; e < 8; e++)
            if (c + e < cols) x[u][e] = s[e];
        }
      }
    }
#pragma unroll
    for (int u = 0; u < 2; u++) {
      const int r = r0 + u;
      if (r >= plane_rows) break;
#pragma unroll
      for (int pl = 0; pl < NP; pl++) {
        uint32_t w[4];
#pragma unroll
        for (int e = 0; e < 4; e++) {
          asm("cvt.rn.bf16x2.f32 %0, %1, %2;" : "=r"(w[e]) : "f"(x[u][2 * e + 1]), "f"(x[u][2 * e]));
          x[u][2 * e] -= __uint_as_float(w[e] << 16);
          x[u][2 * e + 1] -= __uint_as_float(w[e] & 0xFFFF0000u);
        }
        *reinterpret_cast<uint4*>(dst + ((long long)pl * plane_rows + r) * dld + c) = make_uint4(w[0], w[1], w[2], w[3]);
      }
    }
  }
}


__device__ __forceinline__ void split_f16x8(const float (&x)[8], uint4& h1, uint4& h2) {
  uint32_t a[4], b[4];
#pragma unroll
  for (int e = 0; e < 4; e++) {
    const __half2 p = __floats2half2_rn(x[2 * e], x[2 * e + 1]);
    const float2 pf = __half22float2(p);
    const __half2 q = __floats2half2_rn(x[2 * e] - pf.x, x[2 * e + 1] - pf.y);
    a[e] = *reinterpret_cast<const uint32_t*>(&p);
    b[e] = *reinterpret_cast<const uint32_t*>(&q);
  }
  h1 = make_uint4(a[0], a[1], a[2], a[3]);
  h2 = make_uint4(b[0], b[1], b[2], b[3]);
}
__device__ __forceinline__ void load8(const float* __restrict__ s, int c, int cols, bool vec, float (&x)[8]) {
  if (vec && c + 8 <= cols) {
    const float4 v0 = __ldg(reinterpret_cast<const float4*>(s + c));
    const float4 v1 = __ldg(reinterpret_cast<const float4*>(s + c) + 1);
    x[0] = v0.x; x[1] = v0.y; x[2] = v0.z; x[3] = v0.w;
    x[4] = v1.x; x[5] = v1.y; x[6] = v1.z; x[7] = v1.w;
  } else {
#pragma unroll
    for (int e = 0; e < 8; e++) x[e] = c + e < cols ? __ldg(s + c + e) : 0.f;
  }
}

template <int VPL>
__global__ void __launch_bounds__(256) split_f16_rows_kernel(const float* __restrict__ src, long long ld, int rows,
                                                             int cols, float* __restrict__ rmax,
                                                             uint16_t* __restrict__ dst, long long dld, int plane_rows) {
  griddep_launch();
  griddep_wait();
  const int lane = threadIdx.x & 31;
  const int nwarps = (gridDim.x * blockDim.x) >> 5;
  const bool vec = (ld & 3) == 0 && (reinterpret_cast<uintptr_t>(src) & 15) == 0;
  for (int r = (blockIdx.x * blockDim.x + threadIdx.x) >> 5; r < plane_rows; r += nwarps) {
    uint16_t* d1 = dst + (long long)r * dld;
    uint16_t* d2 = dst + ((long long)plane_rows + r) * dld;
    if (r >= rows) {
      for (int c = lane * 8; c < dld; c += 256) {
        *reinterpret_cast<uint4*>(d1 + c) = make_uint4(0, 0, 0, 0);
        *reinterpret_cast<uint4*>(d2 + c) = make_uint4(0, 0, 0, 0);
      }
      continue;
    }
    const float* s = src + (long long)r * ld;
    float mx = 0.f;
    if constexpr (VPL > 0) {
      float x[VPL][8];
#pragma unroll
      for (int j = 0; j < VPL; j++) {
        const int c = (j * 32 + lane) * 8;
#pragma unroll
        for (int e = 0; e < 8; e++) x[j][e] = 0.f;
        if (c < cols) load8(s, c, cols, vec, x[j]);
#pragma unroll
        for (int e = 0; e < 8; e++) mx = fmaxf(mx, fabsf(x[j][e]));
      }
#pragma unroll
      for (int o = 16; o > 0; o >>= 1) mx = fmaxf(mx, __shfl_xor_sync(0xffffffffu, mx, o));
      if (lane == 0) rmax[r] = mx;
      const int ex = -pow2_exp(mx);
#pragma unroll
      for (int j = 0; j < VPL; j++) {
        const int c = (j * 32 + lane) * 8;
        if (c < dld) {
#pragma unroll
          for (int e = 0; e < 8; e++) x[j][e] = mul_pow2(x[j][e], ex);
          uint4 h1, h2;
          split_f16x8(x[j], h1, h2);
          *reinterpret_cast<uint4*>(d1 + c) = h1;
          *reinterpret_cast<uint4*>(d2 + c) = h2;
        }
      }
    } else {
      for (int c0 = lane * 8; c0 < cols; c0 += 1024) {
        float x[4][8];
#pragma unroll
        for (int u = 0; u < 4; u++) {
          const int c = c0 + u * 256;
#pragma unroll
          for (int e = 0; e < 8; e++) x[u][e] = 0.f;
          if (c < cols) load8(s, c, cols, vec, x[u]);
#pragma unroll
          for (int e = 0; e < 8; e++) mx = fmaxf(mx, fabsf(x[u][e]));
        }
      }
#pragma unroll
      for (int o = 16; o > 0; o >>= 1) mx = fmaxf(mx, __shfl_xor_sync(0xffffffffu, mx, o));
      if (lane == 0) rmax[r] = mx;
      const int ex = -pow2_exp(mx);
      for (int c0 = lane * 8; c0 < dld; c0 += 512) {
        float x[2][8];
#pragma unroll
        for (int u = 0; u < 2; u++) {
          const int c = c0 + u * 256;
#pragma unroll
          for (int e = 0; e < 8; e++) x[u][e] = 0.f;
          if (c < cols) load8(s, c, cols, vec, x[u]);
        }
#pragma unroll
        for (int u = 0; u < 2; u++) {
          const int c = c0 + u * 256;
          if (c < dld) {
#pragma unroll
            for (int e = 0; e < 8; e++) x[u][e] = mul_pow2(x[u][e], ex);
            uint4 h1, h2;
            split_f16x8(x[u], h1, h2);
            *reinterpret_cast<uint4*>(d1 + c) = h1;
            *reinterpret_cast<uint4*>(d2 + c) = h2;
          }
        }
      }
    }
  }
}

__global__ void __launch_bounds__(256) col_absmax_kernel(const float* __restrict__ src, long long ld, int rows,
                                                         int cols, unsigned int* __restrict__ out) {
  constexpr int ROWS = 16;
  griddep_launch();
  griddep_wait();
  const int c = blockIdx.x * 1024 + threadIdx.x * 4;
  if (c >= cols) return;
  const int r0 = blockIdx.y * ROWS, r1 = min(r0 + ROWS, rows);
  const bool vec = (ld & 3) == 0 && (reinterpret_cast<uintptr_t>(src) & 15) == 0 && c + 4 <= cols;
  float4 mx = make_float4(0.f, 0.f, 0.f, 0.f);
  if (vec) {
#pragma unroll 16
    for (int r = r0; r < r1; r++) {
      const float4 v = __ldg(reinterpret_cast<const float4*>(src + (long long)r * ld + c));
      mx.x = fmaxf(mx.x, fabsf(v.x)); mx.y = fmaxf(mx.y, fabsf(v.y));
      mx.z = fmaxf(mx.z, fabsf(v.z)); mx.w = fmaxf(mx.w, fabsf(v.w));
    }
  } else {
    for (int r = r0; r < r1; r++) {
      const float* s = src + (long long)r * ld + c;
      mx.x = fmaxf(mx.x, fabsf(s[0]));
      if (c + 1 < cols) mx.y = fmaxf(mx.y, fabsf(s[1]));
      if (c + 2 < cols) mx.z = fmaxf(mx.z, fabsf(s[2]));
      if (c + 3 < cols) mx.w = fmaxf(mx.w, fabsf(s[3]));
    }
  }
  const float m4[4] = {mx.x, mx.y, mx.z, mx.w};
#pragma unroll
  for (int e = 0; e < 4; e++)
    if (c + e < cols && __float_as_uint(m4[e]) > __ldcg(out + c + e)) atomicMax(out + c + e, __float_as_uint(m4[e]));
}

__global__ void __launch_bounds__(256) split_f16_cols_kernel(const float* __restrict__ src, long long ld, int rows,
                                                             int cols, const float* __restrict__ cmax,
                                                             uint16_t* __restrict__ dst, long long dld, int plane_rows,
                                                             float* __restrict__ zero_buf, int zero_n) {
  griddep_launch();
  griddep_wait();
  const int c = (int)(blockIdx.x * 256 + threadIdx.x) * 8;
  if (blockIdx.y == 0 && zero_buf != nullptr) {
#pragma unroll
    for (int e = 0; e < 8; e++)
      if (c + e < zero_n) zero_buf[c + e] = 0.f;
  }
  if (c >= dld) return;
  const bool vec = (ld & 3) == 0 && (reinterpret_cast<uintptr_t>(src) & 15) == 0;
  int ex[8];
#pragma unroll
  for (int e = 0; e < 8; e++) ex[e] = c + e < cols ? -pow2_exp(__ldg(cmax + c + e)) : 0;
  for (int r0 = blockIdx.y * 2; r0 < plane_rows; r0 += gridDim.y * 2) {
    float x[2][8];
#pragma unroll
    for (int u = 0; u < 2; u++) {
      const int r = r0 + u;
#pragma unroll
      for (int e = 0; e < 8; e++) x[u][e] = 0.f;
      if (r < rows) load8(src + (long long)r * ld, c, cols, vec, x[u]);
    }
#pragma unroll
    for (int u = 0; u < 2; u++) {
      const int r = r0 + u;
      if (r >= plane_rows) break;
#pragma unroll
      for (int e = 0; e < 8; e++) x[u][e] = mul_pow2(x[u][e], ex[e]);
      uint4 h1, h2;
      split_f16x8(x[u], h1, h2);
      *reinterpret_cast<uint4*>(dst + (long long)r * dld + c) = h1;
      *reinterpret_cast<uint4*>(dst + ((long long)plane_rows + r) * dld + c) = h2;
    }
  }
}

}
```

### how-to-optimize-gemm_b200/csrc/rowpanel.cuh

```cuda
#pragma once
#include <dlfcn.h>
#include <nccl.h>

namespace {

struct NcclApi {
  void* lib = nullptr;
  bool ok = false;
  ncclResult_t (*Broadcast)(const void*, void*, size_t, ncclDataType_t, int, ncclComm_t, cudaStream_t) = nullptr;
  const char* (*GetErrorString)(ncclResult_t) = nullptr;
  ncclResult_t (*CommCount)(const ncclComm_t, int*) = nullptr;
  ncclResult_t (*CommUserRank)(const ncclComm_t, int*) = nullptr;
  ncclResult_t (*GetUniqueId)(ncclUniqueId*) = nullptr;
  ncclResult_t (*CommInitRank)(ncclComm_t*, int, ncclUniqueId, int) = nullptr;
  ncclResult_t (*CommDestroy)(ncclComm_t) = nullptr;
} g_nccl;
thread_local char t_nccl_err[256] = "";

int nccl_load(const char* path) {
  std::lock_guard<std::mutex> lk(g_mu);
  if (g_nccl.ok) return 0;
  const char* names[3] = {path, "libnccl.so.2", "libnccl.so"};
  for (int i = 0; i < 3 && !g_nccl.lib; i++)
    if (names[i] && names[i][0]) g_nccl.lib = dlopen(names[i], RTLD_NOW | RTLD_GLOBAL);
  if (!g_nccl.lib) { snprintf(t_nccl_err, sizeof t_nccl_err, "dlopen libnccl.so.2: %s", dlerror()); return B200_ERR_NCCL; }
#define NCCL_SYM(field, name)                                                             \
  *reinterpret_cast<void**>(&g_nccl.field) = dlsym(g_nccl.lib, name);                      \
  if (!g_nccl.field) { snprintf(t_nccl_err, sizeof t_nccl_err, "dlsym %s failed", name); return B200_ERR_NCCL; }
  NCCL_SYM(Broadcast, "ncclBroadcast")
  NCCL_SYM(GetErrorString, "ncclGetErrorString")
  NCCL_SYM(CommCount, "ncclCommCount")
  NCCL_SYM(CommUserRank, "ncclCommUserRank")
  NCCL_SYM(GetUniqueId, "ncclGetUniqueId")
  NCCL_SYM(CommInitRank, "ncclCommInitRank")
  NCCL_SYM(CommDestroy, "ncclCommDestroy")
#undef NCCL_SYM
  g_nccl.ok = true;
  return 0;
}
int nccl_check(ncclResult_t r, const char* what) {
  if (r == ncclSuccess) return 0;
  snprintf(t_nccl_err, sizeof t_nccl_err, "%s: %s", what, g_nccl.GetErrorString ? g_nccl.GetErrorString(r) : "?");
  return B200_ERR_NCCL;
}

constexpr int kMaxSlices = 16;

}

struct b200_rowpanel {
  ncclComm_t comm = nullptr;
  int rank = 0, world = 1, dev = -1;
  int m_max = 0, n = 0, k = 0, mode = 0;
  int nslices = 0;
  int trace = 0;
  cudaEvent_t tr[8 + 6 * kMaxSlices] = {};
  int reserve_sms = 0;
  int dynamic_sched = 1;
  int k0[kMaxSlices + 1] = {};
  cudaStream_t comm_stream = nullptr;
  cudaEvent_t ev_start = nullptr, ev_b[kMaxSlices] = {}, ev_done = nullptr;
  uint16_t* a_planes = nullptr; float* a_max = nullptr; long long a_pitch = 0;
  uint16_t* b_planes[kMaxSlices] = {}; float* b_max = nullptr; long long b_pitch = 0; int b_rows[kMaxSlices] = {};
  float *hA = nullptr, *hB = nullptr, *hC = nullptr;
  cudaStream_t h2d = nullptr, comp = nullptr, d2h = nullptr;
  cudaEvent_t ev_hb[kMaxSlices] = {}, ev_in[8] = {}, ev_out[8] = {};
  b200_packed_b* hpb = nullptr;
};

namespace {

void rowpanel_free(b200_rowpanel* rp) {
  if (!rp) return;
  if (rp->a_planes) cudaFree(rp->a_planes);
  if (rp->a_max) cudaFree(rp->a_max);
  for (int j = 0; j < kMaxSlices; j++) if (rp->b_planes[j]) cudaFree(rp->b_planes[j]);
  if (rp->b_max) cudaFree(rp->b_max);
  if (rp->hA) cudaFree(rp->hA);
  if (rp->hB) cudaFree(rp->hB);
  if (rp->hC) cudaFree(rp->hC);
  if (rp->hpb) { pack_release(rp->hpb); delete rp->hpb; }
  for (int j = 0; j < kMaxSlices; j++) { if (rp->ev_b[j]) cudaEventDestroy(rp->ev_b[j]); if (rp->ev_hb[j]) cudaEventDestroy(rp->ev_hb[j]); }
  for (auto& e : rp->tr) if (e) cudaEventDestroy(e);
  for (int j = 0; j < 8; j++) { if (rp->ev_in[j]) cudaEventDestroy(rp->ev_in[j]); if (rp->ev_out[j]) cudaEventDestroy(rp->ev_out[j]); }
  if (rp->ev_start) cudaEventDestroy(rp->ev_start);
  if (rp->ev_done) cudaEventDestroy(rp->ev_done);
  if (rp->comm_stream) cudaStreamDestroy(rp->comm_stream);
  if (rp->h2d) cudaStreamDestroy(rp->h2d);
  if (rp->comp) cudaStreamDestroy(rp->comp);
  if (rp->d2h) cudaStreamDestroy(rp->d2h);
  cudaGetLastError();
  delete rp;
}

inline void rp_mark(b200_rowpanel* rp, int slot, cudaStream_t s) {
  if (!rp->trace) return;
  if (!rp->tr[slot]) cudaEventCreate(&rp->tr[slot]);
  cudaEventRecord(rp->tr[slot], s);
}

#define RP_CK(x) do { cudaError_t e_ = (x); if (e_ != cudaSuccess) { cudaGetLastError(); return (int)e_; } } while (0)

int rowpanel_broadcast(b200_rowpanel* rp, float* dB, int ldb, int n, int root, const cudaEvent_t* wait_per_slice) {
  for (int j = 0; j < rp->nslices; j++) {
    if (wait_per_slice && rp->rank == root) RP_CK(cudaStreamWaitEvent(rp->comm_stream, wait_per_slice[j], 0));
    if (rp->world > 1) {
      float* blk = dB + (size_t)rp->k0[j] * ldb;
      rp_mark(rp, 8 + 6 * j, rp->comm_stream);
      const size_t count = (size_t)(rp->k0[j + 1] - rp->k0[j]) * ldb - (size_t)(ldb - n);
      if (int rc = nccl_check(g_nccl.Broadcast(blk, blk, count, ncclFloat32, root, rp->comm, rp->comm_stream), "ncclBroadcast")) return rc;
    }
    rp_mark(rp, 8 + 6 * j + 1, rp->comm_stream);
    RP_CK(cudaEventRecord(rp->ev_b[j], rp->comm_stream));
  }
  return 0;
}

}

extern "C" {

const char* b200_nccl_last_error(void) { return t_nccl_err; }
int b200_nccl_load(const char* path) { return nccl_load(path); }

int b200_comm_unique_id(void* id128) {
  if (!id128) return B200_ERR_BAD_ARG;
  if (int rc = nccl_load(nullptr)) return rc;
  return nccl_check(g_nccl.GetUniqueId(reinterpret_cast<ncclUniqueId*>(id128)), "ncclGetUniqueId");
}
int b200_comm_init_rank(void** comm_out, const void* id128, int rank, int world) {
  if (!comm_out || !id128 || world < 1 || rank < 0 || rank >= world) return B200_ERR_BAD_ARG;
  if (int rc = nccl_load(nullptr)) return rc;
  ncclUniqueId id;
  memcpy(&id, id128, sizeof id);
  ncclComm_t c = nullptr;
  if (int rc = nccl_check(g_nccl.CommInitRank(&c, world, id, rank), "ncclCommInitRank")) return rc;
  *comm_out = c;
  return 0;
}
int b200_comm_destroy(void* comm) {
  if (!comm) return 0;
  if (int rc = nccl_load(nullptr)) return rc;
  return nccl_check(g_nccl.CommDestroy(reinterpret_cast<ncclComm_t>(comm)), "ncclCommDestroy");
}

int b200_rowpanel_create(b200_rowpanel** out, void* nccl_comm, int m_local_max, int n, int k, int precision_mode,
                         const int* slice_rows, int n_slices) {
  if (!out) return B200_ERR_BAD_ARG;
  *out = nullptr;
  if (m_local_max <= 0 || n <= 0 || k <= 0 || n_slices < 0 || n_slices > kMaxSlices) return B200_ERR_BAD_ARG;
  int rc = ensure_device();
  if (rc) return rc;
  b200_rowpanel* rp = new b200_rowpanel();
  rp->dev = t_ctx->dev;
  rp->comm = reinterpret_cast<ncclComm_t>(nccl_comm);
  if (nccl_comm) {
    if ((rc = nccl_load(nullptr))) { delete rp; return rc; }
    if ((rc = nccl_check(g_nccl.CommCount(rp->comm, &rp->world), "ncclCommCount")) ||
        (rc = nccl_check(g_nccl.CommUserRank(rp->comm, &rp->rank), "ncclCommUserRank"))) { delete rp; return rc; }
  }
  rp->m_max = m_local_max; rp->n = n; rp->k = k;
  rp->mode = resolve_f32_mode(precision_mode);
  if (n_slices > 0 && slice_rows) {
    int acc = 0;
    for (int j = 0; j < n_slices; j++) {
      if (slice_rows[j] <= 0 || (acc & 7)) { delete rp; return B200_ERR_BAD_ARG; }
      rp->k0[j] = acc; acc += slice_rows[j];
    }
    if (acc != k) { delete rp; return B200_ERR_BAD_ARG; }
    rp->k0[n_slices] = k; rp->nslices = n_slices;
  } else if (rp->world == 1 || k < 1024) {
    rp->nslices = 1; rp->k0[0] = 0; rp->k0[1] = k;
  } else {
    const double bytes = (double)k * n * 4.0;
    int ns = (int)((bytes + 268435455.0) / 268435456.0);
    ns = ns < 2 ? 2 : (ns > 8 ? 8 : ns);
    rp->nslices = ns;
    rp->k0[0] = 0;
    if (ns == 2) rp->k0[1] = (int)(((long long)k / 4 + 63) / 64 * 64);
    else for (int j = 1; j < ns; j++) rp->k0[j] = (int)(((long long)k * j / ns + 63) / 64 * 64);
    rp->k0[ns] = k;
  }
#define RP_TRY(x) do { cudaError_t e_ = (x); if (e_ != cudaSuccess) { cudaGetLastError(); rowpanel_free(rp); return (int)e_; } } while (0)
  RP_TRY(cudaStreamCreateWithFlags(&rp->comm_stream, cudaStreamNonBlocking));
  RP_TRY(cudaEventCreateWithFlags(&rp->ev_start, cudaEventDisableTiming));
  RP_TRY(cudaEventCreateWithFlags(&rp->ev_done, cudaEventDisableTiming));
  for (int j = 0; j < rp->nslices; j++) RP_TRY(cudaEventCreateWithFlags(&rp->ev_b[j], cudaEventDisableTiming));
  if (rp->mode == B200_F32_F16X2) {
    rp->a_pitch = f16_pitch(k);
    rp->b_pitch = f16_pitch(n);
    RP_TRY(cudaMalloc(&rp->a_planes, (size_t)2 * m_local_max * rp->a_pitch * 2));
    RP_TRY(cudaMalloc(&rp->a_max, (size_t)m_local_max * 4));
    RP_TRY(cudaMalloc(&rp->b_max, (size_t)rp->nslices * n * 4));
    for (int j = 0; j < rp->nslices; j++) {
      rp->b_rows[j] = f16_b_rows(rp->k0[j + 1] - rp->k0[j]);
      RP_TRY(cudaMalloc(&rp->b_planes[j], (size_t)2 * rp->b_rows[j] * rp->b_pitch * 2));
    }
  }
#undef RP_TRY
  *out = rp;
  return 0;
}

void b200_rowpanel_destroy(b200_rowpanel* rp) { rowpanel_free(rp); }
void b200_rowpanel_trace(b200_rowpanel* rp, int enable) { if (rp) rp->trace = enable; }
int b200_rowpanel_trace_dump(b200_rowpanel* rp, float* out, int cap) {
  if (!rp || !rp->trace || !rp->tr[0]) return 0;
  cudaDeviceSynchronize();
  int n = 0;
  auto get = [&](int slot) { float ms = -1.f; if (rp->tr[slot]) cudaEventElapsedTime(&ms, rp->tr[0], rp->tr[slot]); cudaGetLastError(); return ms; };
  if (n < cap) out[n++] = get(1);
  for (int j = 0; j < rp->nslices; j++)
    for (int e = 0; e < 5; e++) if (n < cap) out[n++] = get(8 + 6 * j + e);
  return n;
}
int b200_rowpanel_set_reserve_sms(b200_rowpanel* rp, int sms) {
  if (!rp || sms < -1 || sms > 64) return B200_ERR_BAD_ARG;
  if (sms == -1) { rp->dynamic_sched = 0; return 0; }
  rp->reserve_sms = sms;
  return 0;
}
int b200_rowpanel_slices(const b200_rowpanel* rp, int* bounds, int cap) {
  if (!rp) return 0;
  for (int j = 0; j <= rp->nslices && j < cap; j++) bounds[j] = rp->k0[j];
  return rp->nslices;
}

int b200_gemm_f32_rowpanel(b200_rowpanel* rp, int m_local, int n, int k, const float* dA, int lda, float* dB,
                           int ldb, float* dC, int ldc, int root, void* stream) {
  if (!rp || n != rp->n || k != rp->k || m_local > rp->m_max || root < 0 || root >= rp->world) return B200_ERR_BAD_ARG;
  int rc = check_args(m_local, n, k, dA, lda, dB, ldb, dC, ldc);
  if (rc < 0) return rc;
  if (!dB || ldb < n) return B200_ERR_BAD_ARG;
  rc = ensure_device();
  if (rc) return rc;
  if (t_ctx->dev != rp->dev) return B200_ERR_BAD_ARG;
  cudaStream_t st = (cudaStream_t)stream;
  rp_mark(rp, 0, st);
  RP_CK(cudaEventRecord(rp->ev_start, st));
  RP_CK(cudaStreamWaitEvent(rp->comm_stream, rp->ev_start, 0));
  if ((rc = rowpanel_broadcast(rp, dB, ldb, n, root, nullptr))) return rc;
  if (m_local == 0) {
    RP_CK(cudaStreamWaitEvent(st, rp->ev_b[rp->nslices - 1], 0));
    return 0;
  }
  if (rp->mode == B200_F32_F16X2) {
    if ((rc = launch_f16_split_rows(dA, lda, m_local, k, rp->a_max, rp->a_planes, rp->a_pitch, m_local, st))) return rc;
    RP_CK(cudaMemsetAsync(rp->b_max, 0, (size_t)rp->nslices * n * 4, st));
    rp_mark(rp, 1, st);
    for (int j = 0; j < rp->nslices; j++) {
      const int kk0 = rp->k0[j], kr = rp->k0[j + 1] - kk0;
      RP_CK(cudaStreamWaitEvent(st, rp->ev_b[j], 0));
      rp_mark(rp, 8 + 6 * j + 2, st);
      float* cmax = rp->b_max + (size_t)j * n;
      if ((rc = launch_f16_split_cols(dB + (size_t)kk0 * ldb, ldb, kr, n, cmax, rp->b_planes[j], rp->b_pitch,
                                      rp->b_rows[j], nullptr, 0, st))) return rc;
      rp_mark(rp, 8 + 6 * j + 3, st);
      const F16Operand oa{rp->a_planes + kk0, rp->a_pitch, m_local, rp->a_max};
      const F16Operand ob{rp->b_planes[j], rp->b_pitch, rp->b_rows[j], cmax};
      const bool corun = rp->world > 1 && j + 1 < rp->nslices;
      t_sm_reserve = corun ? rp->reserve_sms : 0;
      t_dynamic_sched = corun ? rp->dynamic_sched : 0;
      rc = gemm_f16x2_core(m_local, n, kr, oa, ob, dC, ldc, j > 0 ? 1 : 0, st);
      t_sm_reserve = 0; t_dynamic_sched = 0;
      if (rc) return rc;
      rp_mark(rp, 8 + 6 * j + 4, st);
    }
    return 0;
  }
  for (int j = 0; j < rp->nslices; j++) {
    const int kk0 = rp->k0[j], kr = rp->k0[j + 1] - kk0;
    RP_CK(cudaStreamWaitEvent(st, rp->ev_b[j], 0));
    const bool corun = rp->world > 1 && j + 1 < rp->nslices;
    t_sm_reserve = corun ? rp->reserve_sms : 0;
    t_dynamic_sched = corun ? rp->dynamic_sched : 0;
    rc = gemm_f32_impl(m_local, n, kr, dA + kk0, lda, dB + (size_t)kk0 * ldb, ldb, dC, ldc, rp->mode, j > 0 ? 1 : 0, st);
    t_sm_reserve = 0; t_dynamic_sched = 0;
    if (rc) return rc;
  }
  return 0;
}

int b200_gemm_f32_rowpanel_host(b200_rowpanel* rp, int m_local, int n, int k, const float* A, int lda, const float* B,
                                int ldb, float* C, int ldc, int root) {
  if (!rp || n != rp->n || k != rp->k || m_local > rp->m_max || m_local < 0 || root < 0 || root >= rp->world) return B200_ERR_BAD_ARG;
  if (m_local > 0 && (!A || !C || lda < k || ldc < n)) return B200_ERR_BAD_ARG;
  if (rp->rank == root && (!B || ldb < n)) return B200_ERR_BAD_ARG;
  int rc = ensure_device();
  if (rc) return rc;
  if (t_ctx->dev != rp->dev) return B200_ERR_BAD_ARG;
  if (!rp->h2d) {
    RP_CK(cudaStreamCreateWithFlags(&rp->h2d, cudaStreamNonBlocking));
    RP_CK(cudaStreamCreateWithFlags(&rp->comp, cudaStreamNonBlocking));
    RP_CK(cudaStreamCreateWithFlags(&rp->d2h, cudaStreamNonBlocking));
    for (int j = 0; j < rp->nslices; j++) RP_CK(cudaEventCreateWithFlags(&rp->ev_hb[j], cudaEventDisableTiming));
    for (int j = 0; j < 8; j++) {
      RP_CK(cudaEventCreateWithFlags(&rp->ev_in[j], cudaEventDisableTiming));
      RP_CK(cudaEventCreateWithFlags(&rp->ev_out[j], cudaEventDisableTiming));
    }
    RP_CK(cudaMalloc(&rp->hA, (size_t)rp->m_max * k * 4));
    RP_CK(cudaMalloc(&rp->hB, (size_t)k * n * 4));
    RP_CK(cudaMalloc(&rp->hC, (size_t)rp->m_max * n * 4));
  }
  if (rp->rank == root)
    for (int j = 0; j < rp->nslices; j++) {
      const int kk0 = rp->k0[j], kr = rp->k0[j + 1] - kk0;
      RP_CK(cudaMemcpy2DAsync(rp->hB + (size_t)kk0 * n, (size_t)n * 4, B + (size_t)kk0 * ldb, (size_t)ldb * 4, (size_t)n * 4, kr,
                              cudaMemcpyHostToDevice, rp->h2d));
      RP_CK(cudaEventRecord(rp->ev_hb[j], rp->h2d));
    }
  if ((rc = rowpanel_broadcast(rp, rp->hB, n, n, root, rp->ev_hb))) return rc;
  const int blocks = m_local >= 2048 ? 4 : 1;
  const int rows_per = blocks == 1 ? (m_local > 0 ? m_local : 1) : (((m_local + blocks - 1) / blocks + 255) & ~255);
  RP_CK(cudaStreamWaitEvent(rp->comp, rp->ev_b[rp->nslices - 1], 0));
  int nb = 0;
  for (int r0 = 0; r0 < m_local; r0 += rows_per, nb++) {
    const int rows = m_local - r0 < rows_per ? m_local - r0 : rows_per;
    float* dAi = rp->hA + (size_t)r0 * k;
    float* dCi = rp->hC + (size_t)r0 * n;
    RP_CK(cudaMemcpy2DAsync(dAi, (size_t)k * 4, A + (size_t)r0 * lda, (size_t)lda * 4, (size_t)k * 4, rows, cudaMemcpyHostToDevice, rp->h2d));
    RP_CK(cudaMemcpy2DAsync(dCi, (size_t)n * 4, C + (size_t)r0 * ldc, (size_t)ldc * 4, (size_t)n * 4, rows, cudaMemcpyHostToDevice, rp->h2d));
    RP_CK(cudaEventRecord(rp->ev_in[nb], rp->h2d));
    RP_CK(cudaStreamWaitEvent(rp->comp, rp->ev_in[nb], 0));
    if ((rc = gemm_f32_impl(rows, n, k, dAi, k, rp->hB, n, dCi, n, rp->mode, 1, rp->comp))) return rc;
    RP_CK(cudaEventRecord(rp->ev_out[nb], rp->comp));
    RP_CK(cudaStreamWaitEvent(rp->d2h, rp->ev_out[nb], 0));
    RP_CK(cudaMemcpy2DAsync(C + (size_t)r0 * ldc, (size_t)ldc * 4, dCi, (size_t)n * 4, (size_t)n * 4, rows, cudaMemcpyDeviceToHost, rp->d2h));
  }
  RP_CK(cudaStreamSynchronize(rp->d2h));
  RP_CK(cudaStreamSynchronize(rp->comp));
  RP_CK(cudaStreamSynchronize(rp->comm_stream));
  return 0;
}

}
```

Measured before the change: 427,500.

## Fuse f16 split prepasses into one clustered kernel with per-chunk column scales

Replaces the separate row-split, column-absmax (atomicMax) and column-split kernels, plus the aux-stream fork, with one launch. A-row blocks and B column strips share a single grid, and the B strips reduce their column max across a thread-block cluster through distributed shared memory. B scaling becomes per 1024-row K chunk instead of global. The GEMM epilogue rescales accumulators per chunk when exponents differ, and chunk boundaries are aligned to the scale chunks. This removes extra launches, the memset and the second read of B. In exchange it adds exponent checks to the epilogue and may force smaller chunk_k splitting.

```diff
diff --git a/how-to-optimize-gemm_b200/csrc/capi.cu b/how-to-optimize-gemm_b200/csrc/capi.cu
--- a/how-to-optimize-gemm_b200/csrc/capi.cu
+++ b/how-to-optimize-gemm_b200/csrc/capi.cu
@@ -78,12 +78,6 @@
   cudaEvent_t ws_event = nullptr;
   cudaStream_t ws_stream = nullptr;
   bool ws_busy = false;
-  unsigned cmax_slot = 0;
-  float* cmax_buf = nullptr;
-  size_t cmax_cap = 0;
-  int cmax_dirty[2] = {0, 0};
-  cudaStream_t aux = nullptr;
-  cudaEvent_t aux_fork = nullptr, aux_join = nullptr;
   std::mutex host_mu;
   Scratch scr[4];
   HostPipe pipe;
@@ -211,7 +205,6 @@
 }
 
 int g_pdl = 1;
-int g_prepass_fork = 1;
 int g_dynamic_sched = 0;
 template <typename... KArgs, typename... Args>
 cudaError_t launch_pdl(void (*kern)(KArgs...), dim3 grid, dim3 block, size_t smem, cudaStream_t st, int cluster, Args&&... args) {
@@ -302,6 +295,7 @@
   if (p.chunk_kb < 1) p.chunk_kb = 1;
   p.dbg_b_lbo = g_dbg_b_lbo; p.dbg_b_sbo = g_dbg_b_sbo;
   p.row_max = row_max; p.col_max = col_max;
+  p.scale_kb = F16_SCALE_ROWS / Cfg::BK;
   p.accumulate = accumulate;
   p.axpby = t_epi.axpby; p.alpha = t_epi.alpha; p.beta = t_epi.beta;
   p.epi_direct = g_epi_direct;
@@ -508,130 +502,83 @@
 };
 inline long long f16_pitch(int cols) { return ((long long)cols + 7) & ~7LL; }
 inline int f16_b_rows(int k) { return (k + 31) & ~31; }
-
-int launch_f16_split_rows(const float* A, long long lda, int rows, int cols, float* rmax, uint16_t* planes,
-                          long long pitch, int plane_rows, cudaStream_t st) {
-  int blocks = (plane_rows + 7) / 8;
-  const int cap = t_ctx->sms * 16;
-  if (blocks > cap) blocks = cap;
-  if (blocks < 1) blocks = 1;
-  if (cols <= 1024) launch_pdl(split_f16_rows_kernel<4>, dim3(blocks), dim3(256), 0, st, 1, A, (long long)lda, rows, cols, rmax, planes, pitch, plane_rows);
-  else if (cols <= 2048) launch_pdl(split_f16_rows_kernel<8>, dim3(blocks), dim3(256), 0, st, 1, A, (long long)lda, rows, cols, rmax, planes, pitch, plane_rows);
-  else if (cols <= 4096) launch_pdl(split_f16_rows_kernel<16>, dim3(blocks), dim3(256), 0, st, 1, A, (long long)lda, rows, cols, rmax, planes, pitch, plane_rows);
-  else launch_pdl(split_f16_rows_kernel<0>, dim3(blocks), dim3(256), 0, st, 1, A, (long long)lda, rows, cols, rmax, planes, pitch, plane_rows);
+inline size_t f16_b_scales(int k, int n) { return (size_t)((k + F16_SCALE_ROWS - 1) / F16_SCALE_ROWS) * n; }
+
+int launch_f16_split(const F16SplitJob& ja, const F16SplitJob& jb, cudaStream_t st) {
+  int a_blocks = 0;
+  if (ja.rows > 0) {
+    const int rb = 8 / (ja.cols > 2048 && ja.cols <= 4096 ? F16_ROW_WARPS<16> : 1);
+    a_blocks = (ja.plane_rows + rb - 1) / rb;
+    if (a_blocks > t_ctx->sms * 16) a_blocks = t_ctx->sms * 16;
+    a_blocks = (a_blocks + F16_B_CLUSTER - 1) / F16_B_CLUSTER * F16_B_CLUSTER;
+  }
+  const long long b_blocks = jb.rows > 0 ? (long long)F16_B_CLUSTER * ((jb.rows + F16_SCALE_ROWS - 1) / F16_SCALE_ROWS) * ((jb.dld + 127) / 128) : 0;
+  const dim3 grid((unsigned)(a_blocks + b_blocks));
+  if (grid.x == 0) return 0;
+  constexpr int CL = F16_B_CLUSTER;
+  cudaError_t e;
+  if (ja.cols <= 1024) e = launch_pdl(split_f16_ab_kernel<4>, grid, dim3(256), 0, st, CL, ja, a_blocks, jb);
+  else if (ja.cols <= 2048) e = launch_pdl(split_f16_ab_kernel<8>, grid, dim3(256), 0, st, CL, ja, a_blocks, jb);
+  else if (ja.cols <= 4096) e = launch_pdl(split_f16_ab_kernel<16>, grid, dim3(256), 0, st, CL, ja, a_blocks, jb);
+  else e = launch_pdl(split_f16_ab_kernel<0>, grid, dim3(256), 0, st, CL, ja, a_blocks, jb);
+  if (e != cudaSuccess) { cudaGetLastError(); return (int)e; }
   g_launches++;
-  return last_launch_status();
-}
-
-int launch_f16_split_cols(const float* B, long long ldb, int rows, int cols, float* cmax, uint16_t* planes,
-                          long long pitch, int plane_rows, float* zero_buf, int zero_n, cudaStream_t st) {
-  launch_pdl(col_absmax_kernel, dim3((cols + 1023) / 1024, (rows + 15) / 16), dim3(256), 0, st, 1, B, (long long)ldb, rows, cols,
-             reinterpret_cast<unsigned int*>(cmax));
-  const int gx = (int)((pitch + 2047) / 2048);
-  int gy = (t_ctx->sms * 8 + gx - 1) / gx;
-  if (gy > (plane_rows + 1) / 2) gy = (plane_rows + 1) / 2;
-  if (gy < 1) gy = 1;
-  if (zero_buf && zero_n > gx * 2048) {
-    cudaMemsetAsync(zero_buf, 0, (size_t)zero_n * 4, st);
-    zero_buf = nullptr;
-  }
-  launch_pdl(split_f16_cols_kernel, dim3(gx, gy), dim3(256), 0, st, 1, B, (long long)ldb, rows, cols, (const float*)cmax, planes, pitch, plane_rows, zero_buf, zero_n);
-  g_launches += 2;
   return last_launch_status();
 }
 
 int gemm_f16x2_core(int m, int n, int k, const F16Operand& a, const F16Operand& b, float* C, int ldc, int acc,
                     cudaStream_t st) {
   constexpr int NP = 2;
+  int ck = g_split_chunk_k[2];
+  if (ck <= 0 || ck > F16_SCALE_ROWS || F16_SCALE_ROWS % ck != 0) ck = F16_SCALE_ROWS;
   if (use_pair(m, n))
     return launch_tc<KIND_FP16, 256, 6, float, ProdX2, 64, 2>(m, n, k, a.planes, a.pitch, NP * a.plane_rows, a.plane_rows,
                                                               b.planes, b.pitch, NP * b.plane_rows, b.plane_rows, C, ldc, st,
-                                                              "tc_f16x2_2cta_256x256", g_split_chunk_k[2], a.maxv, b.maxv, acc);
+                                                              "tc_f16x2_2cta_256x256", ck, a.maxv, b.maxv, acc);
   const int bn = pick_bn(m, n, true);
   if (bn == 256)
     return launch_tc<KIND_FP16, 256, 4, float, ProdX2, 64>(m, n, k, a.planes, a.pitch, NP * a.plane_rows, a.plane_rows,
                                                            b.planes, b.pitch, NP * b.plane_rows, b.plane_rows, C, ldc, st,
-                                                           "tc_f16x2_128x256", g_split_chunk_k[2], a.maxv, b.maxv, acc);
+                                                           "tc_f16x2_128x256", ck, a.maxv, b.maxv, acc);
   if (bn == 192)
     return launch_tc<KIND_FP16, 192, 4, float, ProdX2, 64>(m, n, k, a.planes, a.pitch, NP * a.plane_rows, a.plane_rows,
                                                            b.planes, b.pitch, NP * b.plane_rows, b.plane_rows, C, ldc, st,
-                                                           "tc_f16x2_128x192", g_split_chunk_k[2], a.maxv, b.maxv, acc);
+                                                           "tc_f16x2_128x192", ck, a.maxv, b.maxv, acc);
   return launch_tc<KIND_FP16, 128, 6, float, ProdX2, 64>(m, n, k, a.planes, a.pitch, NP * a.plane_rows, a.plane_rows,
                                                          b.planes, b.pitch, NP * b.plane_rows, b.plane_rows, C, ldc, st,
-                                                         "tc_f16x2_128x128", g_split_chunk_k[2], a.maxv, b.maxv, acc);
-}
-
-int cmax_reserve(int n, float** cur, float** other, int* other_dirty) {
-  DevCtx* c = t_ctx;
-  if (c->cmax_cap < (size_t)n) {
-    size_t cap = c->cmax_cap ? 2 * c->cmax_cap : 16384;
-    if (cap < (size_t)n) cap = (size_t)n;
-    if (c->cmax_buf) { cudaDeviceSynchronize(); cudaFree(c->cmax_buf); }
-    c->cmax_buf = nullptr; c->cmax_cap = 0;
-    cudaError_t e = cudaMalloc(&c->cmax_buf, 2 * cap * sizeof(float));
-    if (e == cudaSuccess) e = cudaMemset(c->cmax_buf, 0, 2 * cap * sizeof(float));
-    if (e != cudaSuccess) { cudaGetLastError(); return (int)e; }
-    c->cmax_cap = cap;
-    c->cmax_dirty[0] = c->cmax_dirty[1] = 0;
-  }
-  const unsigned slot = c->cmax_slot++ & 1u;
-  *cur = c->cmax_buf + slot * c->cmax_cap;
-  *other = c->cmax_buf + (slot ^ 1u) * c->cmax_cap;
-  *other_dirty = c->cmax_dirty[slot ^ 1u];
-  c->cmax_dirty[slot ^ 1u] = 0;
-  c->cmax_dirty[slot] = n;
-  return 0;
+                                                         "tc_f16x2_128x128", ck, a.maxv, b.maxv, acc);
+}
+
+struct F16Workspace { size_t b_planes, a_max, b_max, total; };
+F16Workspace f16_workspace(int m, int n, int k, bool split_a, bool split_b) {
+  auto up = [](size_t x) { return (x + 1023) & ~(size_t)1023; };
+  F16Workspace w;
+  w.b_planes = up(split_a ? (size_t)2 * m * f16_pitch(k) * 2 : 0);
+  w.a_max = up(w.b_planes + (split_b ? (size_t)2 * f16_b_rows(k) * f16_pitch(n) * 2 : 0));
+  w.b_max = up(w.a_max + (split_a ? (size_t)m * 4 : 0));
+  w.total = w.b_max + (split_b ? f16_b_scales(k, n) * 4 : 0);
+  return w;
 }
 
 int gemm_f32_split_f16(int m, int n, int k, const float* A, int lda, const float* B, int ldb, float* C, int ldc,
                        cudaStream_t st, int acc = 0, const F16Operand* prepA = nullptr, const F16Operand* prepB = nullptr) {
-  constexpr int NP = 2;
+  if (prepA && prepB) return gemm_f16x2_core(m, n, k, *prepA, *prepB, C, ldc, acc, st);
   const long long pka = f16_pitch(k), pnb = f16_pitch(n);
   const int kp = f16_b_rows(k);
-  const size_t a_bytes = prepA ? 0 : (size_t)NP * m * pka * 2, b_bytes = prepB ? 0 : (size_t)NP * kp * pnb * 2;
-  const size_t a_off = (a_bytes + 1023) & ~(size_t)1023;
-  const size_t r_off = (a_off + b_bytes + 1023) & ~(size_t)1023;
-  const size_t total = r_off + (prepA ? 0 : (size_t)m * 4);
-  F16Operand oa, ob;
-  if (prepA && prepB) return gemm_f16x2_core(m, n, k, *prepA, *prepB, C, ldc, acc, st);
+  const F16Workspace w = f16_workspace(m, n, k, !prepA, !prepB);
   std::lock_guard<std::mutex> wlk(t_ctx->ws_mu);
-  if (int rc = split_ws_reserve(total)) return rc;
+  if (int rc = split_ws_reserve(w.total)) return rc;
   ws_acquire(st);
   struct Release { cudaStream_t s; ~Release() { ws_release(s); } } rel{st};
   uint8_t* base = reinterpret_cast<uint8_t*>(t_ctx->ws.p);
-  DevCtx* c = t_ctx;
-  const bool fork = !prepA && !prepB && g_prepass_fork && (double)m * k + (double)k * n >= 4.0e6;
-  cudaStream_t sb = st;
-  if (fork) {
-    if (!c->aux) {
-      if (cudaStreamCreateWithFlags(&c->aux, cudaStreamNonBlocking) != cudaSuccess ||
-          cudaEventCreateWithFlags(&c->aux_fork, cudaEventDisableTiming) != cudaSuccess ||
-          cudaEventCreateWithFlags(&c->aux_join, cudaEventDisableTiming) != cudaSuccess) { cudaGetLastError(); return B200_ERR_NO_DEVICE; }
-    }
-    cudaEventRecord(c->aux_fork, st);
-    cudaStreamWaitEvent(c->aux, c->aux_fork, 0);
-    sb = c->aux;
-  }
-  if (prepB) ob = *prepB;
-  else {
-    uint16_t* pB = reinterpret_cast<uint16_t*>(base + a_off);
-    float *cmax, *other;
-    int other_dirty;
-    if (int rc = cmax_reserve(n, &cmax, &other, &other_dirty)) return rc;
-    if (int rc = launch_f16_split_cols(B, ldb, k, n, cmax, pB, pnb, kp, other, other_dirty, sb)) return rc;
-    ob = F16Operand{pB, pnb, kp, cmax};
-  }
-  if (prepA) oa = *prepA;
-  else {
-    uint16_t* pA = reinterpret_cast<uint16_t*>(base);
-    float* rmax = reinterpret_cast<float*>(base + r_off);
-    if (int rc = launch_f16_split_rows(A, lda, m, k, rmax, pA, pka, m, st)) return rc;
-    oa = F16Operand{pA, pka, m, rmax};
-  }
-  if (fork) {
-    cudaEventRecord(c->aux_join, c->aux);
-    cudaStreamWaitEvent(st, c->aux_join, 0);
-  }
+  uint16_t* pA = reinterpret_cast<uint16_t*>(base);
+  uint16_t* pB = reinterpret_cast<uint16_t*>(base + w.b_planes);
+  float* rmax = reinterpret_cast<float*>(base + w.a_max);
+  float* cmax = reinterpret_cast<float*>(base + w.b_max);
+  const F16Operand oa = prepA ? *prepA : F16Operand{pA, pka, m, rmax};
+  const F16Operand ob = prepB ? *prepB : F16Operand{pB, pnb, kp, cmax};
+  if (int rc = launch_f16_split(prepA ? F16SplitJob{} : F16SplitJob{A, lda, m, k, rmax, pA, pka, m},
+                                prepB ? F16SplitJob{} : F16SplitJob{B, ldb, k, n, cmax, pB, pnb, kp}, st)) return rc;
   return gemm_f16x2_core(m, n, k, oa, ob, C, ldc, acc, st);
 }
 
@@ -772,7 +719,7 @@
 }
 void b200_gemm_debug_set_b_desc(int lbo_bytes, int sbo_bytes) { g_dbg_b_lbo = lbo_bytes; g_dbg_b_sbo = sbo_bytes; }
 void b200_gemm_debug_set_bn(int bn) { g_force_bn = bn; }
-void b200_gemm_debug_set_pdl(int v) { g_pdl = (v & 1) != 0; g_prepass_fork = (v & 2) == 0; }
+void b200_gemm_debug_set_pdl(int v) { g_pdl = (v & 1) != 0; }
 void b200_gemm_debug_set_dynamic_sched(int on) { g_dynamic_sched = on != 0; }
 void b200_gemm_debug_set_cta_group(int cg) { g_force_cg = cg; }
 void b200_gemm_debug_set_split_tail(int on) { g_split_tail = on; }
@@ -805,6 +752,7 @@
   const int mode = resolve_f32_mode(precision_mode);
   const int np = mode == B200_F32_BF16X3 ? 3 : (mode == B200_F32_BF16X2 || mode == B200_F32_F16X2) ? 2 : 0;
   if (!np || m <= 0 || n <= 0 || k <= 0) return 0;
+  if (mode == B200_F32_F16X2) return f16_workspace(m, n, k, true, true).total;
   const size_t a = ((size_t)np * m * plane_pitch(k) * 2 + 1023) & ~(size_t)1023;
   const size_t b = ((size_t)np * b_plane_rows(k) * plane_pitch(n) * 2 + 1023) & ~(size_t)1023;
   return a + b + (size_t)m * 4 + 1024;
@@ -914,14 +862,12 @@
     h->np = 2;
     h->pitch = f16_pitch(cols);
     h->plane_rows = side == 0 ? rows : f16_b_rows(rows);
-    const size_t nmax = side == 0 ? (size_t)rows : (size_t)cols;
+    const size_t nmax = side == 0 ? (size_t)rows : f16_b_scales(rows, cols);
     cudaError_t e = cudaMalloc(&h->planes, (size_t)2 * h->plane_rows * h->pitch * 2);
     if (e == cudaSuccess) e = cudaMalloc(&h->maxv, nmax * 4);
     if (e != cudaSuccess) { cudaGetLastError(); return (int)e; }
-    if (side == 0) return launch_f16_split_rows(d, ld, rows, cols, h->maxv, h->planes, h->pitch, h->plane_rows, st);
-    e = cudaMemsetAsync(h->maxv, 0, nmax * 4, st);
-    if (e != cudaSuccess) { cudaGetLastError(); return (int)e; }
-    return launch_f16_split_cols(d, ld, rows, cols, h->maxv, h->planes, h->pitch, h->plane_rows, nullptr, 0, st);
+    const F16SplitJob j{d, ld, rows, cols, h->maxv, h->planes, h->pitch, h->plane_rows};
+    return side == 0 ? launch_f16_split(j, F16SplitJob{}, st) : launch_f16_split(F16SplitJob{}, j, st);
   }
   h->np = mode == B200_F32_BF16X3 ? 3 : 2;
   h->pitch = plane_pitch(cols);
diff --git a/how-to-optimize-gemm_b200/csrc/gemm_tc.cuh b/how-to-optimize-gemm_b200/csrc/gemm_tc.cuh
--- a/how-to-optimize-gemm_b200/csrc/gemm_tc.cuh
+++ b/how-to-optimize-gemm_b200/csrc/gemm_tc.cuh
@@ -45,6 +45,7 @@
   int* sched_counter;
   const float* row_max;
   const float* col_max;
+  int scale_kb;
   float alpha, beta;
   int axpby;
   int accumulate;
@@ -118,6 +119,25 @@
   return x * exp2i(h) * exp2i(min(e - h, 127));
 }
 
+constexpr int F16_SCALE_ROWS = 1024;
+
+__device__ __forceinline__ int chunk_end(int c0, int kb1, int chunk_kb) { return min((c0 / chunk_kb + 1) * chunk_kb, kb1); }
+
+__device__ __forceinline__ void col_chunk_exps(const TcParams& p, int col, int s0, int s1, int s, int& es, int& E) {
+  es = 0;
+  E = -1000;
+  if (col < p.N) {
+    for (int c = s0; c <= s1; c++) {
+      const float mv = __ldg(p.col_max + (long long)c * p.N + col);
+      const int e = pow2_exp(mv);
+      if (c == s) es = e;
+      const uint32_t ef = (__float_as_uint(mv) >> 23) & 0xFFu;
+      if (ef != 0u && ef != 0xFFu) E = max(E, e);
+    }
+  }
+  if (E == -1000) E = 0;
+}
+
 struct WorkItem { int tile, part, kb0, kb1, nsub, bn; };
 template <int BN>
 __device__ __forceinline__ WorkItem work_item(int w, const TcParams& p, int num_kb) {
@@ -354,11 +374,11 @@
       for (int w = NEXT_ITEM(); w >= 0; w = NEXT_ITEM()) {
        const WorkItem it = work_item<BN>(w, p, num_kb);
        const uint32_t idesc = make_idesc(T::C_FMT, T::AB_FMT, 0, 1, Cfg::TILE_M, it.bn);
-       for (int c0 = it.kb0; c0 < it.kb1; c0 += p.chunk_kb) {
+       for (int c0 = it.kb0, c1; c0 < it.kb1; c0 = c1) {
         mbar_wait(bar_tempty + 8 * as, aph ^ 1);
         tc_fence_after();
         const uint32_t d_tmem = tmem_base + as * Cfg::ACC_STRIDE;
-        const int c1 = min(c0 + p.chunk_kb, it.kb1);
+        c1 = chunk_end(c0, it.kb1, p.chunk_kb);
         for (int kb = c0; kb < c1; kb++) {
           mbar_wait(bar_full + 8 * s, ph);
           tc_fence_after();
@@ -420,17 +440,40 @@
       const uint32_t t_col = (uint32_t)(half * hc);
       float acc[NJ][32];
       const int my_re = (p.row_max != nullptr && m0 + lane < p.M) ? pow2_exp(__ldg(p.row_max + m0 + lane)) : 0;
+      const int s0 = it.kb0 / p.scale_kb, s1 = (it.kb1 - 1) / p.scale_kb;
+      uint32_t mixed = 0;
+      if (p.col_max != nullptr && s1 > s0) {
+#pragma unroll
+        for (int j = 0; j < NJ; j++) {
+          const int col = n0 + j * 32 + lane;
+          if (j < nj && col < p.N) {
+            const int e0 = pow2_exp(__ldg(p.col_max + (long long)s0 * p.N + col));
+            for (int c = s0 + 1; c <= s1; c++)
+              if (pow2_exp(__ldg(p.col_max + (long long)c * p.N + col)) != e0) mixed |= 1u << j;
+          }
+        }
+      }
       bool first = true;
-      for (int c0 = it.kb0; c0 < it.kb1; c0 += p.chunk_kb) {
+      for (int c0 = it.kb0; c0 < it.kb1; c0 = chunk_end(c0, it.kb1, p.chunk_kb)) {
         mbar_wait(bar_tfull + 8 * as, aph);
         tc_fence_after();
         const uint32_t t_addr = tmem_base + ((uint32_t)(q * 32) << 16) + as * Cfg::ACC_STRIDE + t_col;
 #pragma unroll
         for (int j = 0; j < NJ; j++) {
           if (j < nj) {
+            int d = 0;
+            if (__any_sync(0xffffffffu, (mixed >> j) & 1u)) {
+              int es, E;
+              col_chunk_exps(p, n0 + j * 32 + lane, s0, s1, c0 / p.scale_kb, es, E);
+              d = es - E;
+            }
             uint32_t r[32];
             tmem_ld_32x32b_x32(t_addr + j * 32, r);
             tmem_ld_wait();
+            if (__any_sync(0xffffffffu, d != 0)) {
+#pragma unroll
+              for (int i = 0; i < 32; i++) r[i] = __float_as_uint(mul_pow2(__uint_as_float(r[i]), __shfl_sync(0xffffffffu, d, i)));
+            }
             if (first) {
 #pragma unroll
               for (int i = 0; i < 32; i++) acc[j][i] = __uint_as_float(r[i]);
@@ -473,9 +516,17 @@
           const bool vec = p.vec_ok && col + 4 <= p.N;
           int ce[4] = {0, 0, 0, 0};
           if (p.col_max != nullptr) {
-#pragma unroll
-            for (int e = 0; e < 4; e++)
-              if (col + e < p.N) ce[e] = pow2_exp(__ldg(p.col_max + col + e));
+            if (__any_sync(0xffffffffu, (mixed >> j) & 1u)) {
+#pragma unroll
+              for (int e = 0; e < 4; e++) {
+                int es;
+                col_chunk_exps(p, col + e, s0, s1, -1, es, ce[e]);
+              }
+            } else {
+#pragma unroll
+              for (int e = 0; e < 4; e++)
+                if (col + e < p.N) ce[e] = pow2_exp(__ldg(p.col_max + (long long)s0 * p.N + col + e));
+            }
           }
           if (fold && vec) {
 #pragma unroll
@@ -570,7 +621,7 @@
         }
         __syncwarp();
       }
-     for (int c0 = it.kb0; c0 < it.kb1; c0 += p.chunk_kb) {
+     for (int c0 = it.kb0; c0 < it.kb1; c0 = chunk_end(c0, it.kb1, p.chunk_kb)) {
       const bool fold = p.accumulate != 0 || c0 != it.kb0 || it.part > 0 || (p.axpby && p.beta != 0.f);
       const float al = p.axpby ? p.alpha : 1.f;
       const float be = (p.axpby && it.part == 0 && c0 == it.kb0) ? p.beta : 1.f;
@@ -805,18 +856,19 @@
 }
 
 
+__device__ __forceinline__ void split_f16x4(float x0, float x1, float x2, float x3, uint2& h1, uint2& h2) {
+  const __half2 p0 = __floats2half2_rn(x0, x1), p1 = __floats2half2_rn(x2, x3);
+  const float2 f0 = __half22float2(p0), f1 = __half22float2(p1);
+  const __half2 q0 = __floats2half2_rn(x0 - f0.x, x1 - f0.y), q1 = __floats2half2_rn(x2 - f1.x, x3 - f1.y);
+  h1 = make_uint2(*reinterpret_cast<const uint32_t*>(&p0), *reinterpret_cast<const uint32_t*>(&p1));
+  h2 = make_uint2(*reinterpret_cast<const uint32_t*>(&q0), *reinterpret_cast<const uint32_t*>(&q1));
+}
 __device__ __forceinline__ void split_f16x8(const float (&x)[8], uint4& h1, uint4& h2) {
-  uint32_t a[4], b[4];
-#pragma unroll
-  for (int e = 0; e < 4; e++) {
-    const __half2 p = __floats2half2_rn(x[2 * e], x[2 * e + 1]);
-    const float2 pf = __half22float2(p);
-    const __half2 q = __floats2half2_rn(x[2 * e] - pf.x, x[2 * e + 1] - pf.y);
-    a[e] = *reinterpret_cast<const uint32_t*>(&p);
-    b[e] = *reinterpret_cast<const uint32_t*>(&q);
-  }
-  h1 = make_uint4(a[0], a[1], a[2], a[3]);
-  h2 = make_uint4(b[0], b[1], b[2], b[3]);
+  uint2 a0, b0, a1, b1;
+  split_f16x4(x[0], x[1], x[2], x[3], a0, b0);
+  split_f16x4(x[4], x[5], x[6], x[7], a1, b1);
+  h1 = make_uint4(a0.x, a0.y, a1.x, a1.y);
+  h2 = make_uint4(b0.x, b0.y, b1.x, b1.y);
 }
 __device__ __forceinline__ void load8(const float* __restrict__ s, int c, int cols, bool vec, float (&x)[8]) {
   if (vec && c + 8 <= cols) {
@@ -830,55 +882,85 @@
   }
 }
 
+struct F16SplitJob {
+  const float* src; long long ld; int rows, cols;
+  float* maxv;
+  uint16_t* dst; long long dld; int plane_rows;
+};
+
+template <int VPL> constexpr int F16_ROW_WARPS = VPL > 8 ? 2 : 1;
 template <int VPL>
-__global__ void __launch_bounds__(256) split_f16_rows_kernel(const float* __restrict__ src, long long ld, int rows,
-                                                             int cols, float* __restrict__ rmax,
-                                                             uint16_t* __restrict__ dst, long long dld, int plane_rows) {
-  griddep_launch();
-  griddep_wait();
-  const int lane = threadIdx.x & 31;
-  const int nwarps = (gridDim.x * blockDim.x) >> 5;
+__device__ __forceinline__ void split_f16_rows(const F16SplitJob& j, int block, int nblocks, int warp, int lane) {
+  const float* __restrict__ src = j.src;
+  uint16_t* __restrict__ dst = j.dst;
+  const long long ld = j.ld, dld = j.dld;
+  const int rows = j.rows, cols = j.cols, plane_rows = j.plane_rows;
   const bool vec = (ld & 3) == 0 && (reinterpret_cast<uintptr_t>(src) & 15) == 0;
-  for (int r = (blockIdx.x * blockDim.x + threadIdx.x) >> 5; r < plane_rows; r += nwarps) {
-    uint16_t* d1 = dst + (long long)r * dld;
-    uint16_t* d2 = dst + ((long long)plane_rows + r) * dld;
-    if (r >= rows) {
-      for (int c = lane * 8; c < dld; c += 256) {
-        *reinterpret_cast<uint4*>(d1 + c) = make_uint4(0, 0, 0, 0);
-        *reinterpret_cast<uint4*>(d2 + c) = make_uint4(0, 0, 0, 0);
-      }
-      continue;
-    }
-    const float* s = src + (long long)r * ld;
-    float mx = 0.f;
-    if constexpr (VPL > 0) {
-      float x[VPL][8];
-#pragma unroll
-      for (int j = 0; j < VPL; j++) {
-        const int c = (j * 32 + lane) * 8;
-#pragma unroll
-        for (int e = 0; e < 8; e++) x[j][e] = 0.f;
-        if (c < cols) load8(s, c, cols, vec, x[j]);
-#pragma unroll
-        for (int e = 0; e < 8; e++) mx = fmaxf(mx, fabsf(x[j][e]));
+  if constexpr (VPL > 0) {
+    constexpr int WPR = F16_ROW_WARPS<VPL>, RB = 8 / WPR, V = VPL / WPR;
+    __shared__ float s_rmax[8];
+    const int part = warp / RB;
+    for (int r0 = block * RB; r0 < plane_rows; r0 += nblocks * RB) {
+      const int r = r0 + warp % RB;
+      uint16_t* d1 = dst + (long long)r * dld;
+      uint16_t* d2 = dst + ((long long)plane_rows + r) * dld;
+      if (r >= rows && r < plane_rows && part == 0) {
+        for (int c = lane * 8; c < dld; c += 256) {
+          *reinterpret_cast<uint4*>(d1 + c) = make_uint4(0, 0, 0, 0);
+          *reinterpret_cast<uint4*>(d2 + c) = make_uint4(0, 0, 0, 0);
+        }
+      }
+      const bool live = r < rows;
+      const float* s = src + (long long)r * ld;
+      float mx = 0.f;
+      float x[V][8];
+#pragma unroll
+      for (int jj = 0; jj < V; jj++) {
+        const int c = ((part * V + jj) * 32 + lane) * 8;
+#pragma unroll
+        for (int e = 0; e < 8; e++) x[jj][e] = 0.f;
+        if (live && c < cols) load8(s, c, cols, vec, x[jj]);
+#pragma unroll
+        for (int e = 0; e < 8; e++) mx = fmaxf(mx, fabsf(x[jj][e]));
       }
 #pragma unroll
       for (int o = 16; o > 0; o >>= 1) mx = fmaxf(mx, __shfl_xor_sync(0xffffffffu, mx, o));
-      if (lane == 0) rmax[r] = mx;
+      if constexpr (WPR > 1) {
+        if (lane == 0) s_rmax[warp] = mx;
+        __syncthreads();
+#pragma unroll
+        for (int q = 0; q < WPR; q++) mx = fmaxf(mx, s_rmax[warp % RB + q * RB]);
+        __syncthreads();
+      }
+      if (!live) continue;
+      if (lane == 0 && part == 0) j.maxv[r] = mx;
       const int ex = -pow2_exp(mx);
 #pragma unroll
-      for (int j = 0; j < VPL; j++) {
-        const int c = (j * 32 + lane) * 8;
+      for (int jj = 0; jj < V; jj++) {
+        const int c = ((part * V + jj) * 32 + lane) * 8;
         if (c < dld) {
 #pragma unroll
-          for (int e = 0; e < 8; e++) x[j][e] = mul_pow2(x[j][e], ex);
+          for (int e = 0; e < 8; e++) x[jj][e] = mul_pow2(x[jj][e], ex);
           uint4 h1, h2;
-          split_f16x8(x[j], h1, h2);
+          split_f16x8(x[jj], h1, h2);
           *reinterpret_cast<uint4*>(d1 + c) = h1;
           *reinterpret_cast<uint4*>(d2 + c) = h2;
         }
       }
-    } else {
+    }
+  } else {
+    for (int r = block * 8 + warp; r < plane_rows; r += nblocks * 8) {
+      uint16_t* d1 = dst + (long long)r * dld;
+      uint16_t* d2 = dst + ((long long)plane_rows + r) * dld;
+      if (r >= rows) {
+        for (int c = lane * 8; c < dld; c += 256) {
+          *reinterpret_cast<uint4*>(d1 + c) = make_uint4(0, 0, 0, 0);
+          *reinterpret_cast<uint4*>(d2 + c) = make_uint4(0, 0, 0, 0);
+        }
+        continue;
+      }
+      const float* s = src + (long long)r * ld;
+      float mx = 0.f;
       for (int c0 = lane * 8; c0 < cols; c0 += 1024) {
         float x[4][8];
 #pragma unroll
@@ -893,7 +975,7 @@
       }
 #pragma unroll
       for (int o = 16; o > 0; o >>= 1) mx = fmaxf(mx, __shfl_xor_sync(0xffffffffu, mx, o));
-      if (lane == 0) rmax[r] = mx;
+      if (lane == 0) j.maxv[r] = mx;
       const int ex = -pow2_exp(mx);
       for (int c0 = lane * 8; c0 < dld; c0 += 512) {
         float x[2][8];
@@ -921,76 +1003,95 @@
   }
 }
 
-__global__ void __launch_bounds__(256) col_absmax_kernel(const float* __restrict__ src, long long ld, int rows,
-                                                         int cols, unsigned int* __restrict__ out) {
-  constexpr int ROWS = 16;
+constexpr int F16_B_CLUSTER = 8;
+__device__ __forceinline__ void split_f16_cols_strip(const F16SplitJob& j, int strip, int rank, int warp, int lane) {
+  constexpr int RPW = F16_SCALE_ROWS / F16_B_CLUSTER / 8;
+  __shared__ __align__(16) float s_part[8][128];
+  __shared__ __align__(16) float s_blk[128];
+  const int groups = (int)((j.dld + 127) / 128);
+  const int chunk = strip / groups;
+  const int c0 = (strip - chunk * groups) * 128 + lane * 4;
+  const int r0 = chunk * F16_SCALE_ROWS + rank * (F16_SCALE_ROWS / F16_B_CLUSTER) + warp;
+  const int nv = c0 < j.cols ? min(RPW, max(0, (j.rows - r0 + 7) >> 3)) : 0;
+  const int ns = c0 < j.dld ? min(RPW, max(0, (j.plane_rows - r0 + 7) >> 3)) : 0;
+  const bool vec = c0 + 4 <= j.cols && (j.ld & 3) == 0 && (reinterpret_cast<uintptr_t>(j.src) & 15) == 0;
+  const float* __restrict__ s = j.src + (long long)r0 * j.ld + c0;
+  const long long sstep = 8 * j.ld;
+  float4 x[RPW];
+#pragma unroll
+  for (int i = 0; i < RPW; i++) {
+    x[i] = make_float4(0.f, 0.f, 0.f, 0.f);
+    if (i < nv) {
+      if (vec) {
+        x[i] = __ldcs(reinterpret_cast<const float4*>(s));
+      } else {
+        x[i].x = __ldcs(s);
+        if (c0 + 1 < j.cols) x[i].y = __ldcs(s + 1);
+        if (c0 + 2 < j.cols) x[i].z = __ldcs(s + 2);
+        if (c0 + 3 < j.cols) x[i].w = __ldcs(s + 3);
+      }
+    }
+    s += sstep;
+  }
+  float4 mx = make_float4(0.f, 0.f, 0.f, 0.f);
+#pragma unroll
+  for (int i = 0; i < RPW; i++) {
+    mx.x = fmaxf(mx.x, fabsf(x[i].x)); mx.y = fmaxf(mx.y, fabsf(x[i].y));
+    mx.z = fmaxf(mx.z, fabsf(x[i].z)); mx.w = fmaxf(mx.w, fabsf(x[i].w));
+  }
+  *reinterpret_cast<float4*>(&s_part[warp][lane * 4]) = mx;
+  __syncthreads();
+  if (threadIdx.x < 128) {
+    float m = 0.f;
+#pragma unroll
+    for (int w = 0; w < 8; w++) m = fmaxf(m, s_part[w][threadIdx.x]);
+    s_blk[threadIdx.x] = m;
+  }
+  cluster_sync();
+#pragma unroll
+  for (int r = 0; r < F16_B_CLUSTER; r++) {
+    float4 v;
+    asm volatile("ld.shared::cluster.v4.f32 {%0, %1, %2, %3}, [%4];"
+                 : "=f"(v.x), "=f"(v.y), "=f"(v.z), "=f"(v.w) : "r"(mapa(smem_u32(&s_blk[lane * 4]), r)) : "memory");
+    mx.x = fmaxf(mx.x, v.x); mx.y = fmaxf(mx.y, v.y); mx.z = fmaxf(mx.z, v.z); mx.w = fmaxf(mx.w, v.w);
+  }
+  cluster_sync();
+  if (rank == 0 && warp == 0) {
+    float* out = j.maxv + (long long)chunk * j.cols + c0;
+    const float m4[4] = {mx.x, mx.y, mx.z, mx.w};
+#pragma unroll
+    for (int e = 0; e < 4; e++)
+      if (c0 + e < j.cols) out[e] = m4[e];
+  }
+  float f1[4], f2[4];
+  const float m4[4] = {mx.x, mx.y, mx.z, mx.w};
+#pragma unroll
+  for (int e = 0; e < 4; e++) {
+    const int ex = -pow2_exp(m4[e]);
+    f1[e] = exp2i(ex >> 1);
+    f2[e] = exp2i(min(ex - (ex >> 1), 127));
+  }
+  uint16_t* __restrict__ d = j.dst + (long long)r0 * j.dld + c0;
+  const long long dstep = 8 * j.dld, plane = (long long)j.plane_rows * j.dld;
+#pragma unroll
+  for (int i = 0; i < RPW; i++) {
+    if (i < ns) {
+      uint2 h1, h2;
+      split_f16x4(x[i].x * f1[0] * f2[0], x[i].y * f1[1] * f2[1], x[i].z * f1[2] * f2[2], x[i].w * f1[3] * f2[3], h1, h2);
+      *reinterpret_cast<uint2*>(d) = h1;
+      *reinterpret_cast<uint2*>(d + plane) = h2;
+    }
+    d += dstep;
+  }
+}
+
+template <int VPL>
+__global__ void __launch_bounds__(256, 2) split_f16_ab_kernel(const F16SplitJob ja, int a_blocks, const F16SplitJob jb) {
   griddep_launch();
   griddep_wait();
-  const int c = blockIdx.x * 1024 + threadIdx.x * 4;
-  if (c >= cols) return;
-  const int r0 = blockIdx.y * ROWS, r1 = min(r0 + ROWS, rows);
-  const bool vec = (ld & 3) == 0 && (reinterpret_cast<uintptr_t>(src) & 15) == 0 && c + 4 <= cols;
-  float4 mx = make_float4(0.f, 0.f, 0.f, 0.f);
-  if (vec) {
-#pragma unroll 16
-    for (int r = r0; r < r1; r++) {
-      const float4 v = __ldg(reinterpret_cast<const float4*>(src + (long long)r * ld + c));
-      mx.x = fmaxf(mx.x, fabsf(v.x)); mx.y = fmaxf(mx.y, fabsf(v.y));
-      mx.z = fmaxf(mx.z, fabsf(v.z)); mx.w = fmaxf(mx.w, fabsf(v.w));
-    }
-  } else {
-    for (int r = r0; r < r1; r++) {
-      const float* s = src + (long long)r * ld + c;
-      mx.x = fmaxf(mx.x, fabsf(s[0]));
-      if (c + 1 < cols) mx.y = fmaxf(mx.y, fabsf(s[1]));
-      if (c + 2 < cols) mx.z = fmaxf(mx.z, fabsf(s[2]));
-      if (c + 3 < cols) mx.w = fmaxf(mx.w, fabsf(s[3]));
-    }
-  }
-  const float m4[4] = {mx.x, mx.y, mx.z, mx.w};
-#pragma unroll
-  for (int e = 0; e < 4; e++)
-    if (c + e < cols && __float_as_uint(m4[e]) > __ldcg(out + c + e)) atomicMax(out + c + e, __float_as_uint(m4[e]));
-}
-
-__global__ void __launch_bounds__(256) split_f16_cols_kernel(const float* __restrict__ src, long long ld, int rows,
-                                                             int cols, const float* __restrict__ cmax,
-                                                             uint16_t* __restrict__ dst, long long dld, int plane_rows,
-                                                             float* __restrict__ zero_buf, int zero_n) {
-  griddep_launch();
-  griddep_wait();
-  const int c = (int)(blockIdx.x * 256 + threadIdx.x) * 8;
-  if (blockIdx.y == 0 && zero_buf != nullptr) {
-#pragma unroll
-    for (int e = 0; e < 8; e++)
-      if (c + e < zero_n) zero_buf[c + e] = 0.f;
-  }
-  if (c >= dld) return;
-  const bool vec = (ld & 3) == 0 && (reinterpret_cast<uintptr_t>(src) & 15) == 0;
-  int ex[8];
-#pragma unroll
-  for (int e = 0; e < 8; e++) ex[e] = c + e < cols ? -pow2_exp(__ldg(cmax + c + e)) : 0;
-  for (int r0 = blockIdx.y * 2; r0 < plane_rows; r0 += gridDim.y * 2) {
-    float x[2][8];
-#pragma unroll
-    for (int u = 0; u < 2; u++) {
-      const int r = r0 + u;
-#pragma unroll
-      for (int e = 0; e < 8; e++) x[u][e] = 0.f;
-      if (r < rows) load8(src + (long long)r * ld, c, cols, vec, x[u]);
-    }
-#pragma unroll
-    for (int u = 0; u < 2; u++) {
-      const int r = r0 + u;
-      if (r >= plane_rows) break;
-#pragma unroll
-      for (int e = 0; e < 8; e++) x[u][e] = mul_pow2(x[u][e], ex[e]);
-      uint4 h1, h2;
-      split_f16x8(x[u], h1, h2);
-      *reinterpret_cast<uint4*>(dst + (long long)r * dld + c) = h1;
-      *reinterpret_cast<uint4*>(dst + ((long long)plane_rows + r) * dld + c) = h2;
-    }
-  }
-}
-
-}
+  const int warp = threadIdx.x >> 5, lane = threadIdx.x & 31;
+  if ((int)blockIdx.x < a_blocks) split_f16_rows<VPL>(ja, (int)blockIdx.x, a_blocks, warp, lane);
+  else split_f16_cols_strip(jb, ((int)blockIdx.x - a_blocks) / F16_B_CLUSTER, (int)cluster_ctarank(), warp, lane);
+}
+
+}
diff --git a/how-to-optimize-gemm_b200/csrc/rowpanel.cuh b/how-to-optimize-gemm_b200/csrc/rowpanel.cuh
--- a/how-to-optimize-gemm_b200/csrc/rowpanel.cuh
+++ b/how-to-optimize-gemm_b200/csrc/rowpanel.cuh
@@ -191,7 +191,9 @@
     rp->b_pitch = f16_pitch(n);
     RP_TRY(cudaMalloc(&rp->a_planes, (size_t)2 * m_local_max * rp->a_pitch * 2));
     RP_TRY(cudaMalloc(&rp->a_max, (size_t)m_local_max * 4));
-    RP_TRY(cudaMalloc(&rp->b_max, (size_t)rp->nslices * n * 4));
+    size_t b_scales = 0;
+    for (int j = 0; j < rp->nslices; j++) b_scales += f16_b_scales(rp->k0[j + 1] - rp->k0[j], n);
+    RP_TRY(cudaMalloc(&rp->b_max, b_scales * 4));
     for (int j = 0; j < rp->nslices; j++) {
       rp->b_rows[j] = f16_b_rows(rp->k0[j + 1] - rp->k0[j]);
       RP_TRY(cudaMalloc(&rp->b_planes[j], (size_t)2 * rp->b_rows[j] * rp->b_pitch * 2));
@@ -245,16 +247,17 @@
     return 0;
   }
   if (rp->mode == B200_F32_F16X2) {
-    if ((rc = launch_f16_split_rows(dA, lda, m_local, k, rp->a_max, rp->a_planes, rp->a_pitch, m_local, st))) return rc;
-    RP_CK(cudaMemsetAsync(rp->b_max, 0, (size_t)rp->nslices * n * 4, st));
+    if ((rc = launch_f16_split(F16SplitJob{dA, lda, m_local, k, rp->a_max, rp->a_planes, rp->a_pitch, m_local}, F16SplitJob{}, st)))
+      return rc;
     rp_mark(rp, 1, st);
+    float* cmax = rp->b_max;
     for (int j = 0; j < rp->nslices; j++) {
       const int kk0 = rp->k0[j], kr = rp->k0[j + 1] - kk0;
+      if (j > 0) cmax += f16_b_scales(rp->k0[j] - rp->k0[j - 1], n);
       RP_CK(cudaStreamWaitEvent(st, rp->ev_b[j], 0));
       rp_mark(rp, 8 + 6 * j + 2, st);
-      float* cmax = rp->b_max + (size_t)j * n;
-      if ((rc = launch_f16_split_cols(dB + (size_t)kk0 * ldb, ldb, kr, n, cmax, rp->b_planes[j], rp->b_pitch,
-                                      rp->b_rows[j], nullptr, 0, st))) return rc;
+      if ((rc = launch_f16_split(F16SplitJob{}, F16SplitJob{dB + (size_t)kk0 * ldb, ldb, kr, n, cmax, rp->b_planes[j], rp->b_pitch,
+                                                            rp->b_rows[j]}, st))) return rc;
       rp_mark(rp, 8 + 6 * j + 3, st);
       const F16Operand oa{rp->a_planes + kk0, rp->a_pitch, m_local, rp->a_max};
       const F16Operand ob{rp->b_planes[j], rp->b_pitch, rp->b_rows[j], cmax};
```

Measured after the change: 431,000, median of 6. Within noise of the previous version (+0.8%).
